# GBATZOLIS/conditional_score_diffusion

Hardware: AMD Instinct MI355X
Metric: images/sec for 1000-step PC sampling, ddpm_paired_SR3 score net of celebA_SR3_160 (BASELINE configs[1]), 160x160 (higher is better)
Workload: dtype f16x3 (every operand carried as hi + lo fp16 = 22 significand bits, 3 MFMAs per product, f32 accumulate; f32-class: the per-op test tolerance is the f32 kernel's, network error 1.9e-6 vs the reference); 1 GPU; BASELINE configs[1]: celebA_SR3_160 (ddpm_paired_SR3, nf=96, ch_mult (1,1,2,2,3,3), attn 20/10/5), 1000-step PC (reverse_diffusion + langevin, snr 0.15), batch 64 per GPU, random-init weights, synthetic LR inputs; images_per_gpu=64, global_batch=64, noise=on-device Philox4x32-10, precision_mode=fp16x3

## Files before the change

### conditional_score_diffusion_amd/csrc/conv_ff.h

```cpp
#pragma once
#include <stdlib.h>

#include <type_traits>

#include "conv_f16_kernel.h"

namespace csd {

typedef unsigned int uint4f __attribute__((ext_vector_type(4)));
typedef int int8v __attribute__((ext_vector_type(8)));
typedef short short2v __attribute__((ext_vector_type(2)));

#define FF_THREADS 256
#define FF_TILE 16
#define FF_PW 18
#define FF_NPATCH (FF_PW * FF_PW)
#define FF_PSB 64
#define FF_RS (FF_PW * FF_PSB + 16)
#define FF_PATCH_BYTES (FF_PW * FF_RS)

struct ConvFFArgs {
  ConvArgs a;
  int B, H, W, C0, C1, Cout;
  int tiles_x, tpi, n_groups, nblocks;
  int nstage;
  int abl;
};

__device__ __forceinline__ void ff_barrier() {
  asm volatile("" ::: "memory");
  __builtin_amdgcn_s_waitcnt(0xC07F);
  __builtin_amdgcn_s_barrier();
  asm volatile("" ::: "memory");
}

template <int N>
__device__ __forceinline__ void ff_wait_vm() {
  asm volatile("s_waitcnt vmcnt(%0)" ::"n"(N) : "memory");
}

template <int NS, int NT>
struct FFCfg {
  static constexpr int KC = NS == 1 ? 32 : 16;
  static constexpr int KSUB = NS == 1 ? 2 : 1;
  static constexpr int STEPS = KSUB * 9;
  static constexpr int TG = NS == 1 ? 2 : 1;
  static constexpr int GPS = STEPS / TG;
  static constexpr int SB = NT * NS * 1024;
  static constexpr int GB = TG * SB;
  static constexpr int GL = GB / 1024;
  static constexpr int R = 5;
  static constexpr int G4 = KC / 4;
  static constexpr int NDMA = 1;
  static constexpr int GLW = GL / NDMA;
  static constexpr int LOADERS = (4 - NDMA) * 64;
  static constexpr int NSLOT = (FF_NPATCH * G4 + LOADERS - 1) / LOADERS;
  static constexpr int PPJ = LOADERS / G4;
  static constexpr size_t LDS = 2 * (size_t)FF_PATCH_BYTES + (size_t)R * GB + 2 * FF_NPATCH * sizeof(int);
};

int convfx_launch(const ConvFFArgs& k, int nt, hipStream_t s);
bool convxk_supported(const ConvFFArgs& k, int nt);
int convxk_launch(const ConvFFArgs& k, int nt, hipStream_t s);

}
```

### conditional_score_diffusion_amd/csrc/conv_xk.hip

```cpp
#include "conv_ff.h"

#include <utility>

namespace csd {

#define XW_THREADS 256
#define XW_RS (32 * 64 + 16)
#define XW_PATCH_BYTES (FF_PW * XW_RS)
#define XW_NU 162

template <int NT_>
struct XKCfg {
  static constexpr int NT = NT_;
  static constexpr int NA = 4 * NT;
  static constexpr int GP = 3 * NA;
  static constexpr int TAPB = 4 * NT * 2 * 1024;
  static constexpr int STB = 3 * TAPB;
  static constexpr int WPT = 2 * NT;
  static constexpr int XTOG = 65536;
  static constexpr int SLOTB = NT * 1024;
  static constexpr int OFF_X23 = XW_PATCH_BYTES, OFF_DUMMY = OFF_X23 + 8 * SLOTB, OFF_Y0 = XTOG + XW_PATCH_BYTES, OFF_Y8 = 2 * XTOG;
  static constexpr int OFF_RED = OFF_Y8 + 8 * SLOTB;
  static constexpr size_t LDS = (size_t)OFF_RED + 4 * NT * 32 * 2 * sizeof(float);
  static_assert(OFF_DUMMY + 3072 <= XTOG && OFF_Y0 + 8 * SLOTB <= OFF_DUMMY + XTOG && OFF_DUMMY + XTOG + 3072 <= OFF_Y8 && 8 * SLOTB <= XW_PATCH_BYTES &&
                    LDS <= 160 * 1024,
                "conv_xk: LDS map");
};

template <class F, int... I>
__device__ __forceinline__ void xk_static_for_impl(F&& f, std::integer_sequence<int, I...>) {
  (f(std::integral_constant<int, I>{}), ...);
}
template <int N, class F>
__device__ __forceinline__ void xk_static_for(F&& f) {
  xk_static_for_impl(static_cast<F&&>(f), std::make_integer_sequence<int, N>{});
}

typedef unsigned int xk_u4 __attribute__((ext_vector_type(4)));

__device__ __forceinline__ int xk_pack_f16(float a, float b) {
  typedef float f2 __attribute__((ext_vector_type(2)));
  typedef _Float16 h2 __attribute__((ext_vector_type(2)));
  return __builtin_bit_cast(int, __builtin_convertvector(f2{a, b}, h2));
}
template <bool HIGH>
__device__ __forceinline__ float xk_lo(int hp, float v) {
  float r;
  if constexpr (HIGH) asm("v_fma_mix_f32 %0, %1, -1.0, %2 op_sel:[1,0,0] op_sel_hi:[1,0,0]" : "=v"(r) : "v"(hp), "v"(v));
  else asm("v_fma_mix_f32 %0, %1, -1.0, %2 op_sel_hi:[1,0,0]" : "=v"(r) : "v"(hp), "v"(v));
  return r;
}

#define XW_FENCE() __builtin_amdgcn_sched_barrier(0)
#define XW_SADD(x, y) asm volatile("s_add_u32 %0, %0, %1" : "+s"(x) : "s"(y) : "scc")
#define XW_PIN(a) asm volatile("" : "+v"(a))
#ifndef XK_ABL
#define XK_ABL 0
#endif
#ifdef CSD_FF_TUNE
#define XW_WALL(i) do { if (a_dbg && tid == 0) a_dbg[blockIdx.x * 32 + (i)] = wall_clock64(); } while (0)
#else
#define XW_WALL(i) do { } while (0)
#endif

template <int NT>
struct XKSched {
  static constexpr int PB = 4 * NT, GP = 3 * PB, WPT = 2 * NT;
  static constexpr bool rd_xl(int g) { return g < PB && g % NT == NT - 1; }
  static constexpr bool rd_xh(int g) { return g >= 2 * PB && g % NT == NT - 1; }
  static constexpr bool slot_req(int g) { return g == 0; }
  static constexpr bool ld_w(int g) { return g >= PB && g < PB + WPT; }
  static constexpr int fixed(int g) { return (rd_xl(g) ? 1 : 0) + (rd_xh(g) ? 1 : 0) + (ld_w(g) ? 1 : 0) + (slot_req(g) ? 3 : 0); }
  static constexpr int wgt(int g) { return 14 - 3 * fixed(g) > 2 ? 14 - 3 * fixed(g) : 2; }
  static constexpr int cum(int g) { int s = 0; for (int h = 0; h < g; ++h) s += wgt(h); return s; }
  static constexpr int first_op(int n, int g) { return (int)(((long long)n * cum(g)) / cum(GP)); }
};

template <int NT_, bool NORM, bool RES>
__global__ __launch_bounds__(XW_THREADS, 1) void conv_xk_kernel(const char* __restrict__ g_wpack, const ConvFFArgs k) {
  using C = XKCfg<NT_>;
  using S = XKSched<NT_>;
  constexpr int NT = C::NT, NA = C::NA, GP = C::GP, TAPB = C::TAPB, STB = C::STB, WPT = C::WPT, PB = S::PB;
  constexpr int OFF_RED = C::OFF_RED, OFF_DUMMY = C::OFF_DUMMY, XTOG = C::XTOG, SLOTB = C::SLOTB;
  extern __shared__ __attribute__((aligned(16))) char smem[];

  const float* const a_src0 = k.a.src0;
  const float* const a_src1 = k.a.src1;
  const float* const a_bias = k.a.bias;
  const float* const a_temb = k.a.temb;
  const float* const a_res = k.a.res;
  float* const a_out = k.a.out;
  double* const a_stats = k.a.stats;
  const int a_temb_stride = k.a.temb_stride, a_out_stride = k.a.out_stride, a_out_coff = k.a.out_coff;
  const float a_out_scale = k.a.out_scale;
  const int kH = k.H, kW = k.W, kC0 = k.C0, kC1 = k.C1, kCout = k.Cout, k_tiles_x = k.tiles_x, k_tpi = k.tpi,
            k_n_groups = k.n_groups, k_nblocks = k.nblocks, NS = k.nstage;
  const int Cin = kC0 + kC1;

  const int tid = threadIdx.x;
  const int lane = tid & 63;
  const int wave = __builtin_amdgcn_readfirstlane(tid >> 6);
  const int kh = lane >> 5, p32 = lane & 31, lg = lane & 3, ul = lane >> 2;
#ifdef CSD_FF_TUNE
  long long* const a_dbg = k.a.dbg;
#endif
  XW_WALL(30);

  const int xcd = blockIdx.x & 7, wj = blockIdx.x >> 3, wstride = gridDim.x >> 3;
  const int xq = k_nblocks >> 3, xr = k_nblocks & 7;
  const int x_start = xcd < xr ? xcd * (xq + 1) : xr * (xq + 1) + (xcd - xr) * xq, x_len = xq + (xcd < xr ? 1 : 0);
  const int n_my = x_len > wj ? (x_len - wj + wstride - 1) / wstride : 0;
  if (n_my == 0) return;
  struct Tile { int ng, b, ty0, tx0, tile; };
  auto tile_at = [&](int it) __attribute__((always_inline)) {
    Tile t;
    it = it < n_my ? it : n_my - 1;
    const int w = x_start + wj + it * wstride;
    t.ng = w % k_n_groups;
    t.tile = w / k_n_groups;
    t.b = t.tile / k_tpi;
    const int tin = t.tile - t.b * k_tpi;
    t.ty0 = (tin / k_tiles_x) * FF_TILE;
    t.tx0 = (tin - (tin / k_tiles_x) * k_tiles_x) * FF_TILE;
    return t;
  };

  auto fresh_lane = [&]() __attribute__((always_inline)) { int l = lane; asm volatile("" : "+v"(l)); return l; };
  constexpr unsigned OOB = 0x80000000u;
  constexpr int RSRC_FLAGS = 0x00020000;
  constexpr float NLOG2E = -1.4426950408889634f;
  const float ka = (NORM ? -0.6931471805599453f / C16_WSCALE : 1.0f / C16_WSCALE) * a_out_scale;

  int s_dst[3];
#pragma unroll
  for (int j = 0; j < 3; ++j) {
    const int U = 15 * (4 * j + wave) + ul;
    const int Uc = U < XW_NU ? U : XW_NU - 1;
    const int pr = Uc / 9, u = Uc - pr * 9;
    const bool writer = U < XW_NU && ul < 15 && u < 8;
    const int rec = pr * XW_RS + u * 64 + lg * 8;
    const int dummy = OFF_DUMMY + ul * 64 + lg * 8;
    s_dst[j] = writer ? rec : dummy;
  }
  struct Geom { int p[3]; };
  auto geom_of = [&](const Tile& t) __attribute__((always_inline)) {
    Geom g;
    const int ulf = fresh_lane() >> 2;
#pragma unroll
    for (int j = 0; j < 3; ++j) {
      const int U = 15 * (4 * j + wave) + ulf;
      const int Uc = U < XW_NU ? U : XW_NU - 1;
      const int pr = Uc / 9, u = Uc - pr * 9;
      const int y = t.ty0 - 1 + pr, xa = t.tx0 - 1 + 2 * u;
      const bool iny = (unsigned)y < (unsigned)kH && U < XW_NU;
      const bool ina = iny && (unsigned)xa < (unsigned)kW, inb = iny && (unsigned)(xa + 1) < (unsigned)kW;
      g.p[j] = (ina ? y * kW + xa : inb ? y * kW + xa + 1 : 0) | (ina ? (int)0x80000000 : 0) | (inb ? 0x40000000 : 0) |
               (ina && inb ? 0x20000000 : 0);
    }
    return g;
  };
  const int nb_addr = ((lane + 4) & 63) * 4;

  const int xbase = (p32 >> 3) * XW_RS + (p32 & 7) * 64 + kh * 16 + wave * 512;
  int xb_cur = xbase, xb_nxt = xbase + XTOG;

  xk_u4 pfa[3], pfb[3];
  xk_u4 scn, shn;
  float msc[4], msh[4];
  __amdgpu_buffer_rsrc_t srcL;
  int strideL = 0, soffL = 0;
  auto src_of = [&](const Tile& t, int st) __attribute__((always_inline)) {
    const int cb = st * 16;
    const bool s1 = cb >= kC0;
    const int Cs = s1 ? kC1 : kC0;
    const float* base = (s1 ? a_src1 : a_src0) + (size_t)t.b * kH * kW * Cs;
    srcL = __builtin_amdgcn_make_buffer_rsrc(const_cast<float*>(base), 0, OOB, RSRC_FLAGS);
    strideL = Cs * 4;
    soffL = (s1 ? cb - kC0 : cb) * 4;
  };
  auto req_a = [&](int j, const Geom& g) __attribute__((always_inline)) {
    if (!(XK_ABL & 16)) pfa[j] = __builtin_amdgcn_raw_buffer_load_b128(srcL, (XK_ABL & 8192) ? (unsigned)(tid * 16 + j * 8192) : __umul24((XK_ABL & 4096) ? (g.p[j] & 255) : g.p[j], strideL) + lg * 16, soffL, 0);
  };
  auto req_b = [&](int j, const Geom& g) __attribute__((always_inline)) {
    if (!(XK_ABL & 16)) pfb[j] = __builtin_amdgcn_raw_buffer_load_b128(srcL, (XK_ABL & 8192) ? (unsigned)(tid * 16 + j * 8192 + 4096) : __umul24(((XK_ABL & 4096) ? (g.p[j] & 255) : g.p[j]) + ((g.p[j] >> 29) & 1), strideL) + lg * 16, soffL, 0);
  };
  const __amdgpu_buffer_rsrc_t nsc_r = __builtin_amdgcn_make_buffer_rsrc(const_cast<float*>(NORM ? k.a.nscale : a_src0), 0, OOB, RSRC_FLAGS);
  const __amdgpu_buffer_rsrc_t nsh_r = __builtin_amdgcn_make_buffer_rsrc(const_cast<float*>(NORM ? k.a.nshift : a_src0), 0, OOB, RSRC_FLAGS);
  auto req_norm = [&](const Tile& t, int st) __attribute__((always_inline)) {
    if constexpr (NORM) {
      const int so = (t.b * Cin + st * 16) * 4;
      scn = __builtin_amdgcn_raw_buffer_load_b128(nsc_r, (unsigned)(lg * 16), so, 0);
      shn = __builtin_amdgcn_raw_buffer_load_b128(nsh_r, (unsigned)(lg * 16), so, 0);
    }
  };
  auto cvt_prep_half = [&](int h) __attribute__((always_inline)) {
    if constexpr (NORM) {
#pragma unroll
      for (int q = 2 * h; q < 2 * h + 2; ++q) {
        msc[q] = __uint_as_float(scn[q]) * NLOG2E;
        msh[q] = __uint_as_float(shn[q]) * NLOG2E;
      }
      asm volatile("" : "+v"(msc[2 * h]), "+v"(msc[2 * h + 1]), "+v"(msh[2 * h]), "+v"(msh[2 * h + 1]));
    }
  };
  const __amdgpu_buffer_rsrc_t w_r = __builtin_amdgcn_make_buffer_rsrc(const_cast<char*>(g_wpack), 0, OOB, RSRC_FLAGS);
  const int wvoff = lane * 16 + wave * (WPT * 1024);
  int w_run = 0;
  const int c_tapb = TAPB;
  auto w_begin = [&](int wso) __attribute__((always_inline)) { w_run = wso; };
  auto w_next_tap = [&]() __attribute__((always_inline)) { XW_SADD(w_run, c_tapb); };

  constexpr int NPH = NORM ? 7 : 2, NPRE = 8 * NPH, NPOST = 24, NMATH = NPRE + 2 * NPOST;
  struct PreOrder {
    int val[8 * 7], ph[8 * 7];
    constexpr PreOrder(int nph) : val{}, ph{} {
      int n = 0;
      for (int d = 0; d < nph + 7; ++d)
        for (int i = 0; i < 8; ++i)
          if (d - i >= 0 && d - i < nph) { val[n] = i; ph[n] = d - i; ++n; }
    }
  };
  constexpr PreOrder PRE(NPH);
  float cv[8], ce[8], cn[8], cd[4][2], cl[4][2];
  int chp[4][2], clp[4][2];
  auto math_op = [&](auto j_tag, auto o_tag, const Geom& g) __attribute__((always_inline)) {
    constexpr int j = decltype(j_tag)::value, ol = decltype(o_tag)::value;
    if (XK_ABL & 1) return;
    if constexpr (ol < NPRE) {
      constexpr int i = PRE.val[ol], c = i & 3, o = PRE.ph[ol] + (NORM ? 0 : 5);
      if constexpr (o == 0) {
        const float x = __uint_as_float(i < 4 ? pfa[j][c] : pfb[j][c]);
        cv[i] = fmaf(x, msc[c], msh[c]);
        XW_PIN(cv[i]);
      } else if constexpr (o == 1) {
        ce[i] = (XK_ABL & 1024) ? cv[i] * 1.5f : __builtin_amdgcn_exp2f(cv[i]);
        XW_PIN(ce[i]);
      } else if constexpr (o == 2) {
        ce[i] = 1.0f + ce[i];
        XW_PIN(ce[i]);
      } else if constexpr (o == 3) {
        ce[i] = (XK_ABL & 1024) ? ce[i] * 0.7f : __builtin_amdgcn_rcpf(ce[i]);
        XW_PIN(ce[i]);
      } else if constexpr (o == 4) {
        cv[i] = cv[i] * ce[i];
        XW_PIN(cv[i]);
      } else if constexpr (o == 5) {
        const int m = (i < 4 ? g.p[j] : g.p[j] << 1) >> 31;
        const int raw = NORM ? __float_as_int(cv[i]) : (int)(i < 4 ? pfa[j][c] : pfb[j][c]);
        cv[i] = __int_as_float(raw & m);
        XW_PIN(cv[i]);
      } else {
        if (XK_ABL & 512) { cn[i] = cv[i] * 0.5f; XW_PIN(cn[i]); }
        else cn[i] = __int_as_float(__builtin_amdgcn_ds_bpermute(nb_addr, __float_as_int(cv[i])));
      }
    } else {
      constexpr int hh = (ol - NPRE) / NPOST, o = (ol - NPRE) % NPOST;
      if constexpr (o < 8) {
        constexpr int kc = o >> 1, c = o & 1, ca = 2 * hh + c, cb = 4 + ca;
        if constexpr (kc == 0) cd[0][c] = cv[ca] - cn[ca];
        else if constexpr (kc == 1) cd[1][c] = cv[cb] + cn[ca];
        else if constexpr (kc == 2) cd[2][c] = cn[ca] - cv[cb];
        else cd[3][c] = cv[cb] - cn[cb];
        XW_PIN(cd[kc][c]);
      } else if constexpr (o < 12) {
        constexpr int kc = o - 8;
        if (XK_ABL & 2048) { chp[kc][hh] = __float_as_int(cd[kc][0]); clp[kc][hh] = __float_as_int(cd[kc][1]); return; }
        chp[kc][hh] = xk_pack_f16(cd[kc][0], cd[kc][1]);
        XW_PIN(chp[kc][hh]);
      } else if constexpr (o < 20) {
        if (XK_ABL & 2048) return;
        constexpr int kc = (o - 12) >> 1, c = (o - 12) & 1;
        if constexpr (c == 0) cl[kc][0] = xk_lo<false>(chp[kc][hh], cd[kc][0]);
        else cl[kc][1] = xk_lo<true>(chp[kc][hh], cd[kc][1]);
        XW_PIN(cl[kc][c]);
      } else {
        if (XK_ABL & 2048) return;
        constexpr int kc = o - 20;
        clp[kc][hh] = xk_pack_f16(cl[kc][0], cl[kc][1]);
        XW_PIN(clp[kc][hh]);
      }
    }
  };
  auto write_op = [&](auto j_tag, auto o_tag) __attribute__((always_inline)) {
    constexpr int j = decltype(j_tag)::value, o = decltype(o_tag)::value;
    if (XK_ABL & (1 | 256)) return;
    constexpr int kc = o & 3, pl = o >> 2;
    char* const rec = smem + s_dst[j] + kc * 512 + pl * 32;
    if constexpr (pl == 0) *reinterpret_cast<int2*>(rec) = make_int2(chp[kc][0], chp[kc][1]);
    else *reinterpret_cast<int2*>(rec) = make_int2(clp[kc][0], clp[kc][1]);
  };
  auto reqs_op = [&](auto j_tag, auto o_tag, const Geom& g) __attribute__((always_inline)) {
    constexpr int j = decltype(j_tag)::value, o = decltype(o_tag)::value;
    if constexpr (o == 0) req_a(j, g);
    else req_b(j, g);
  };
  using J0 = std::integral_constant<int, 0>;
  using J1 = std::integral_constant<int, 1>;
  using J2 = std::integral_constant<int, 2>;
  constexpr int NFULL = NMATH + 8;
  auto full_op = [&](auto j_tag, auto o_tag, const Geom& gm, const Geom& gr) __attribute__((always_inline)) {
    constexpr int o = decltype(o_tag)::value;
    if constexpr (o < NMATH) math_op(j_tag, o_tag, gm);
    else write_op(j_tag, std::integral_constant<int, o - NMATH>{});
  };

  half8 xh[4], xl[4], w0[WPT], w1[WPT], w2[WPT];
  auto rd_x = [&](half8& dst, int xb, int r, int m, int pl) __attribute__((always_inline)) {
    if (XK_ABL & 4) return;
    dst = *reinterpret_cast<const half8*>(smem + xb + (4 * m + r) * XW_RS + pl * 32);
  };
  auto ld_w = [&](half8& dst, int i) __attribute__((always_inline)) {
    if (XK_ABL & 2) return;
    dst = __builtin_bit_cast(half8, __builtin_amdgcn_raw_buffer_load_b128(w_r, (unsigned)(wvoff + i * 1024), w_run, 0));
  };

  floatx16 acc[4][NT];
#define XK_MFMA_AV(ACC, A, B) asm volatile("v_mfma_f32_32x32x16_f16 %0, %1, %2, %0" : "+a"(ACC) : "a"(A), "v"(B))
#define XK_MFMA_AA(ACC, A, B) asm volatile("v_mfma_f32_32x32x16_f16 %0, %1, %2, %0" : "+a"(ACC) : "a"(A), "a"(B))
  auto mm0 = [&](int p, int i) __attribute__((always_inline)) {
    const int m = i / NT, nt = i - m * NT, wi = 2 * nt + (p == 2 ? 1 : 0);
    if (p == 0) XK_MFMA_AV(acc[m][nt], xl[m], w0[wi]); else XK_MFMA_AV(acc[m][nt], xh[m], w0[wi]);
  };
  auto mm1 = [&](int p, int i) __attribute__((always_inline)) {
    const int m = i / NT, nt = i - m * NT, wi = 2 * nt + (p == 2 ? 1 : 0);
    if (p == 0) XK_MFMA_AV(acc[m][nt], xl[m], w1[wi]); else XK_MFMA_AV(acc[m][nt], xh[m], w1[wi]);
  };
  auto mm2 = [&](int p, int i) __attribute__((always_inline)) {
    const int m = i / NT, nt = i - m * NT, wi = 2 * nt + (p == 2 ? 1 : 0);
    if (p == 0) XK_MFMA_AV(acc[m][nt], xl[m], w2[wi]); else XK_MFMA_AV(acc[m][nt], xh[m], w2[wi]);
  };
  auto mm_first = [&](int i) __attribute__((always_inline)) {
    const int m = i / NT, nt = i - m * NT;
    asm volatile("v_mfma_f32_32x32x16_f16 %0, %1, %2, 0" : "=a"(acc[m][nt]) : "a"(xl[m]), "v"(w0[2 * nt]));
  };
  auto tie_acc_done = [&]() __attribute__((always_inline)) {
    static_assert(NT == 3 || NT == 2, "conv_xk: 96- or 64-cout groups");
    if constexpr (NT == 3)
      asm volatile("s_nop 15\n\ts_nop 7"
                   : "+a"(acc[0][0]), "+a"(acc[0][1]), "+a"(acc[0][2]), "+a"(acc[1][0]), "+a"(acc[1][1]), "+a"(acc[1][2]), "+a"(acc[2][0]),
                     "+a"(acc[2][1]), "+a"(acc[2][2]), "+a"(acc[3][0]), "+a"(acc[3][1]), "+a"(acc[3][2]));
    else
      asm volatile("s_nop 15\n\ts_nop 7"
                   : "+a"(acc[0][0]), "+a"(acc[0][1]), "+a"(acc[1][0]), "+a"(acc[1][1]), "+a"(acc[2][0]), "+a"(acc[2][1]), "+a"(acc[3][0]),
                     "+a"(acc[3][1]));
  };

  float rs[4][8][NT];
  float bv[NT], tv[NT];
  __amdgpu_buffer_rsrc_t res_r, out_r;
  unsigned res_voff = 0, out_voff = 0;
  bool e_valid = true;
  int e_tile = 0, e_ng = 0;
  const int res_col = kCout * 4, res_row = (kW - 7) * kCout * 4, out_col = a_out_stride * 4, out_row = (kW - 7) * a_out_stride * 4;
  int res_run = 0;
  const __amdgpu_buffer_rsrc_t bias_r = __builtin_amdgcn_make_buffer_rsrc(const_cast<float*>(a_bias ? a_bias : a_src0), 0, a_bias ? OOB : 0u, RSRC_FLAGS);
  auto epi_setup = [&](const Tile& t) __attribute__((always_inline)) {
    const size_t tile_pix = (size_t)t.b * kH * kW + (size_t)t.ty0 * kW + t.tx0;
    out_r = __builtin_amdgcn_make_buffer_rsrc(a_out + tile_pix * a_out_stride + a_out_coff, 0, OOB, RSRC_FLAGS);
    e_tile = t.tile; e_ng = t.ng;
    if constexpr (RES) {
      res_r = __builtin_amdgcn_make_buffer_rsrc(const_cast<float*>(a_res + tile_pix * kCout), 0, OOB, RSRC_FLAGS);
      res_run = 0;
    }
  };
  auto epi_loads = [&](const Tile& t) __attribute__((always_inline)) {
    const int lf = fresh_lane();
    const int c_lane = t.ng * NT * 32 + (lf & 31);
    e_valid = (t.ty0 + 4 * wave < kH) && (t.tx0 + 8 * (lf >> 5) < kW);
    out_voff = e_valid ? (unsigned)((4 * wave * kW + 8 * (lf >> 5)) * a_out_stride + c_lane) * 4u : OOB;
    if constexpr (RES) res_voff = e_valid ? (unsigned)((4 * wave * kW + 8 * (lf >> 5)) * kCout + c_lane) * 4u : OOB;
    const __amdgpu_buffer_rsrc_t tb_r = __builtin_amdgcn_make_buffer_rsrc(const_cast<float*>(a_temb ? a_temb + (size_t)t.b * a_temb_stride : a_src0), 0,
                                                                           a_temb ? OOB : 0u, RSRC_FLAGS);
#pragma unroll
    for (int nt = 0; nt < NT; ++nt) {
      bv[nt] = __uint_as_float(__builtin_amdgcn_raw_buffer_load_b32(bias_r, (unsigned)(c_lane + nt * 32) * 4u, 0, 0));
      tv[nt] = __uint_as_float(__builtin_amdgcn_raw_buffer_load_b32(tb_r, (unsigned)(c_lane + nt * 32) * 4u, 0, 0));
    }
  };
  auto req_res = [&](int e) __attribute__((always_inline)) {
    if constexpr (RES) {
      if (XK_ABL & 32) return;
      const int idx = e / NT, nt = e - idx * NT;
      rs[idx >> 3][idx & 7][nt] = __uint_as_float(__builtin_amdgcn_raw_buffer_load_b32(res_r, res_voff + nt * 128, res_run, 0));
      if (nt == NT - 1 && idx < 31) {
        if ((idx & 7) != 7) XW_SADD(res_run, res_col);
        else XW_SADD(res_run, res_row);
      }
    }
  };
  float* const red = reinterpret_cast<float*>(smem + OFF_RED);
  int ex_dead = XTOG;
  auto epilogue = [&]() __attribute__((always_inline)) {
    if constexpr (RES) {
#pragma unroll
      for (int e = 8 * NT; e < 32 * NT; ++e) req_res(e);
    }
    tie_acc_done();
    const int lf = fresh_lane();
    const int l16 = lf * 16;
    const int txX01 = ex_dead + wave * SLOTB + l16, txX23 = C::OFF_X23 + wave * SLOTB + l16;
    const int txY0 = C::OFF_Y0 + wave * SLOTB + l16, txY8 = C::OFF_Y8 + wave * SLOTB + l16;
    const int rxX = (wave < 2 ? ex_dead + wave * 4 * SLOTB : C::OFF_X23 + (wave - 2) * 4 * SLOTB) + l16;
    const int rxY = (wave < 2 ? C::OFF_Y0 + wave * 4 * SLOTB : C::OFF_Y8 + (wave - 2) * 4 * SLOTB) + l16;
    float ps[NT][4], pq[NT][4];
#pragma unroll
    for (int nt = 0; nt < NT; ++nt)
#pragma unroll
      for (int q = 0; q < 4; ++q) ps[nt][q] = pq[nt][q] = 0.f;
    int out_run = 0;
    typedef float xk_f4 __attribute__((ext_vector_type(4)));
    auto send_block = [&](int row, int d) __attribute__((always_inline)) {
      const int tx = (row & 1) ? ((d < 2 ? txY0 : txY8) + (d & 1) * 4 * SLOTB) : ((d < 2 ? txX01 : txX23) + (d & 1) * 4 * SLOTB);
#pragma unroll
      for (int nt = 0; nt < NT; ++nt)
        if (!(XK_ABL & 128))
          *reinterpret_cast<xk_f4*>(smem + tx + nt * 1024) =
              xk_f4{acc[d][nt][4 * row], acc[d][nt][4 * row + 1], acc[d][nt][4 * row + 2], acc[d][nt][4 * row + 3]};
    };
#pragma unroll
    for (int row = 0; row < ((XK_ABL & 524288) ? 0 : 4); ++row) {
      if (row == 0) {
#pragma unroll
        for (int d = 0; d < 4; ++d) send_block(0, d);
      }
      if (!(XK_ABL & 65536)) ff_barrier();
      xk_f4 mv[4][NT];
#pragma unroll
      for (int c = 0; c < 4; ++c)
#pragma unroll
        for (int nt = 0; nt < NT; ++nt) {
          if (XK_ABL & 131072) mv[c][nt] = xk_f4{acc[c][nt][4 * row], acc[c][nt][4 * row + 1], acc[c][nt][4 * row + 2], acc[c][nt][4 * row + 3]};
          else mv[c][nt] = *reinterpret_cast<const xk_f4*>(smem + ((row & 1) ? rxY : rxX) + c * SLOTB + nt * 1024);
        }
#pragma unroll
      for (int jj = 0; jj < 4; ++jj) {
        float y1[NT];
#pragma unroll
        for (int nt = 0; nt < NT; ++nt) {
          const float bs = (bv[nt] + tv[nt]) * a_out_scale;
          const float m0 = mv[0][nt][jj], m1 = mv[1][nt][jj], m2 = mv[2][nt][jj], m3 = mv[3][nt][jj];
          const float y0 = (m0 + m1) + m2;
          y1[nt] = (m1 - m2) - m3;
          float v;
          if constexpr (RES) v = fmaf(y0, ka, fmaf(rs[row][2 * jj][nt], a_out_scale, bs));
          else v = fmaf(y0, ka, bs);
          if (!(XK_ABL & 8)) __builtin_amdgcn_raw_buffer_store_b32(__float_as_uint(v), out_r, out_voff + nt * 128, out_run, 0);
          if (!(XK_ABL & 262144)) { ps[nt][(jj & 1) * 2] += v; pq[nt][(jj & 1) * 2] = fmaf(v, v, pq[nt][(jj & 1) * 2]); }
        }
        XW_SADD(out_run, out_col);
#pragma unroll
        for (int nt = 0; nt < NT; ++nt) {
          const float bs = (bv[nt] + tv[nt]) * a_out_scale;
          float v;
          if constexpr (RES) v = fmaf(y1[nt], ka, fmaf(rs[row][2 * jj + 1][nt], a_out_scale, bs));
          else v = fmaf(y1[nt], ka, bs);
          if (!(XK_ABL & 8)) __builtin_amdgcn_raw_buffer_store_b32(__float_as_uint(v), out_r, out_voff + nt * 128, out_run, 0);
          if (!(XK_ABL & 262144)) { ps[nt][(jj & 1) * 2 + 1] += v; pq[nt][(jj & 1) * 2 + 1] = fmaf(v, v, pq[nt][(jj & 1) * 2 + 1]); }
        }
        if (jj != 3) XW_SADD(out_run, out_col);
        else if (row != 3) XW_SADD(out_run, out_row);
        XW_FENCE();
        if (row < 3) send_block(row + 1, jj);
        XW_FENCE();
      }
    }
    if (a_stats) {
      const int tidf = wave * 64 + lf;
      float vs[NT], vq[NT];
#pragma unroll
      for (int nt = 0; nt < NT; ++nt) {
        vs[nt] = (ps[nt][0] + ps[nt][1]) + (ps[nt][2] + ps[nt][3]);
        vq[nt] = (pq[nt][0] + pq[nt][1]) + (pq[nt][2] + pq[nt][3]);
        vs[nt] = e_valid ? vs[nt] : 0.f;
        vq[nt] = e_valid ? vq[nt] : 0.f;
        vs[nt] += __shfl_xor(vs[nt], 32);
        vq[nt] += __shfl_xor(vq[nt], 32);
        if (lf < 32) {
          red[(wave * NT * 32 + nt * 32 + lf) * 2 + 0] = vs[nt];
          red[(wave * NT * 32 + nt * 32 + lf) * 2 + 1] = vq[nt];
        }
      }
      ff_barrier();
      if (tidf < NT * 32) {
        double sm = 0.0, sq = 0.0;
#pragma unroll
        for (int wv = 0; wv < 4; ++wv) {
          sm += (double)red[(wv * NT * 32 + tidf) * 2 + 0];
          sq += (double)red[(wv * NT * 32 + tidf) * 2 + 1];
        }
        double* dst = a_stats + ((size_t)e_tile * kCout + e_ng * NT * 32 + tidf) * 2;
        dst[0] = sm;
        dst[1] = sq;
      }
    }
  };

  Tile tc = tile_at(0), tn = tile_at(1);
  Geom gc = geom_of(tc), gn = gc;
  const int NSTB = (Cin / 16) * STB;

  src_of(tc, 0);
#pragma unroll
  for (int j = 0; j < 3; ++j) { req_a(j, gc); req_b(j, gc); }
  req_norm(tc, 0);
  w_begin(tc.ng * NSTB);
  {
    cvt_prep_half(0); cvt_prep_half(1);
    req_norm(tc, 1);
    src_of(tc, 1);
    xk_static_for<NFULL>([&](auto o) __attribute__((always_inline)) { full_op(J0{}, o, gc, gc); });
    req_a(0, gc); req_b(0, gc);
    xk_static_for<NFULL>([&](auto o) __attribute__((always_inline)) { full_op(J1{}, o, gc, gc); });
    req_a(1, gc); req_b(1, gc);
    xk_static_for<NFULL>([&](auto o) __attribute__((always_inline)) { full_op(J2{}, o, gc, gc); });
    req_a(2, gc); req_b(2, gc);
#pragma unroll
    for (int j = 0; j < 3; ++j) s_dst[j] ^= XTOG;
    cvt_prep_half(0); cvt_prep_half(1);
    xk_static_for<NMATH>([&](auto o) __attribute__((always_inline)) { math_op(J0{}, o, gc); });
#pragma unroll
    for (int i = 0; i < WPT; ++i) ld_w(w0[i], i);
    w_next_tap();
#pragma unroll
    for (int i = 0; i < WPT; ++i) ld_w(w1[i], i);
    w_next_tap();
  }
  ff_barrier();
#pragma unroll
  for (int m = 0; m < 4; ++m) { rd_x(xh[m], xb_cur, 0, m, 0); rd_x(xl[m], xb_cur, 0, m, 1); }

  auto unit = [&](auto pos_tag, auto first_tag, int s) __attribute__((always_inline)) {
    constexpr int POS = decltype(pos_tag)::value;
    constexpr bool FIRST = decltype(first_tag)::value;
    const Tile& tx = POS == 2 ? tn : tc;
    const Tile& tl = POS >= 1 ? tn : tc;
    const Geom& gx = POS == 2 ? gn : gc;
    const Geom& gl = POS >= 1 ? gn : gc;
    const int sl = POS == 0 ? s + 2 : POS - 1;
    xk_static_for<3>([&](auto r_tag) __attribute__((always_inline)) {
      constexpr int R = decltype(r_tag)::value;
      XW_FENCE();
      if constexpr (R == 2) { if (!(XK_ABL & 64)) ff_barrier(); }
      XW_FENCE();
      if constexpr (R == 0) src_of(tl, sl);
      if constexpr (R == 1 && POS == 2) w_begin(tn.ng * NSTB);
      constexpr int NOPS = R == 0 ? 8 + NFULL : R == 1 ? NFULL : 2 + NMATH;
      xk_static_for<GP>([&](auto g_tag) __attribute__((always_inline)) {
        constexpr int g = decltype(g_tag)::value;
        XW_FENCE();
        if constexpr (FIRST && R == 0 && g < NA) mm_first(g);
        else if constexpr (R == 0) mm0(g / NA, g % NA);
        else if constexpr (R == 1) mm1(g / NA, g % NA);
        else mm2(g / NA, g % NA);
        XW_FENCE();
        if constexpr (S::rd_xl(g)) rd_x(xl[g / NT], R == 2 ? xb_nxt : xb_cur, (R + 1) % 3, g / NT, 1);
        if constexpr (S::rd_xh(g)) rd_x(xh[(g - 2 * PB) / NT], R == 2 ? xb_nxt : xb_cur, (R + 1) % 3, (g - 2 * PB) / NT, 0);
        if constexpr (S::slot_req(g)) { req_a(R, gl); req_b(R, gl); }
        if constexpr (S::ld_w(g)) {
          if constexpr (R == 0) ld_w(w2[g - PB], g - PB);
          else if constexpr (R == 1) ld_w(w0[g - PB], g - PB);
          else ld_w(w1[g - PB], g - PB);
          if constexpr (g == PB + WPT - 1) w_next_tap();
        }
        if constexpr (R == 0 && g == 2 && POS == 1) epi_setup(tc);
        if constexpr (R == 1 && g == PB + PB / 2) req_norm(tl, sl);
        if constexpr (R == 2 && POS == 2 && g == PB) epi_loads(tc);
        constexpr int o0 = S::first_op(NOPS, g), o1 = S::first_op(NOPS, g + 1);
        xk_static_for<o1 - o0>([&](auto d_tag) __attribute__((always_inline)) {
          constexpr int o = o0 + decltype(d_tag)::value;
          if constexpr (R == 0) {
            if constexpr (o < 8) write_op(J0{}, std::integral_constant<int, o>{});
            else full_op(J1{}, std::integral_constant<int, o - 8>{}, gx, gl);
          } else if constexpr (R == 1) {
            full_op(J2{}, std::integral_constant<int, o>{}, gx, gl);
          } else {
            if constexpr (o < 2) cvt_prep_half(o);
            else math_op(J0{}, std::integral_constant<int, o - 2>{}, gl);
          }
        });
        if constexpr (RES && POS == 2 && R == 2 && g >= 2 * PB) {
          constexpr int per = (8 * NT + PB - 1) / PB;
#pragma unroll
          for (int e = (g - 2 * PB) * per; e < (g - 2 * PB + 1) * per && e < 8 * NT; ++e) req_res(e);
        }
      });
    });
    XW_FENCE();
#pragma unroll
    for (int j = 0; j < 3; ++j) s_dst[j] ^= XTOG;
    xb_cur ^= XTOG;
    xb_nxt ^= XTOG;
    ex_dead ^= XTOG;
  };
  using P0 = std::integral_constant<int, 0>;
  using P1 = std::integral_constant<int, 1>;
  using P2 = std::integral_constant<int, 2>;
  using Yes = std::true_type;
  using No = std::false_type;

  for (int it = 0; it < n_my; ++it) {
#ifdef CSD_FF_TUNE
    if (it == 1) XW_WALL(28);
    if (it == 2) XW_WALL(29);
    if (it == 1 && a_dbg && tid == 0) a_dbg[blockIdx.x * 32 + 26] = clock64();
    if (it == 2 && a_dbg && tid == 0) a_dbg[blockIdx.x * 32 + 27] = clock64();
#endif
    unit(P0{}, Yes{}, 0);
    for (int s = 1; s + 2 < NS; ++s) unit(P0{}, No{}, s);
    gn = geom_of(tn);
    unit(P1{}, No{}, NS - 2);
    unit(P2{}, No{}, NS - 1);
    epilogue();
    tc = tn;
    gc = gn;
    tn = tile_at(it + 2);
  }
  XW_WALL(31);
}

template <int NT, bool NORM, bool RES>
static int launch_xk(const ConvFFArgs& k, hipStream_t s) {
  auto kern = conv_xk_kernel<NT, NORM, RES>;
  CSD_SET_MAX_LDS_ONCE(kern);
  const int n_cu = device_cu_count8();
  const int grid = k.nblocks < n_cu ? (k.nblocks + 7) / 8 * 8 : n_cu;
  hipLaunchKernelGGL(kern, dim3(grid), dim3(XW_THREADS), XKCfg<NT>::LDS, s, reinterpret_cast<const char*>(k.a.wpack), k);
  CSD_LAUNCH_CHECK();
  return CSD_OK;
}

bool convxk_supported(const ConvFFArgs& k, int nt) { return (nt == 3 || nt == 2) && k.nstage >= 3; }

int convxk_launch(const ConvFFArgs& k, int nt, hipStream_t s) {
  const bool norm = k.a.nscale != nullptr, res = k.a.res != nullptr;
  if (nt == 2) {
    if (norm) return res ? launch_xk<2, true, true>(k, s) : launch_xk<2, true, false>(k, s);
    return res ? launch_xk<2, false, true>(k, s) : launch_xk<2, false, false>(k, s);
  }
  if (norm) return res ? launch_xk<3, true, true>(k, s) : launch_xk<3, true, false>(k, s);
  return res ? launch_xk<3, false, true>(k, s) : launch_xk<3, false, false>(k, s);
}

}
```

Before: 1.619 images/sec.

## Add half-height tile path to conv_xk for 8-row remainder strips

The conv_xk kernel body moves into an include file instantiated for MT=4 (full 16-row tiles) and MT=2 (half-height tiles). When H mod 16 is 8, as at the 40/10 resolutions, the last tile row is handled by separate workgroups running a half-height walk with a rescheduled op sequence and two prefetch slots. The launcher splits the grid between full and half workers using a cost model. This is meant to avoid computing padded rows that are masked out, at the cost of a more complex schedule, a larger binary and a risk of load imbalance between the two groups.

```diff
diff --git a/conditional_score_diffusion_amd/csrc/conv_ff.h b/conditional_score_diffusion_amd/csrc/conv_ff.h
--- a/conditional_score_diffusion_amd/csrc/conv_ff.h
+++ b/conditional_score_diffusion_amd/csrc/conv_ff.h
@@ -25,6 +25,7 @@
   int tiles_x, tpi, n_groups, nblocks;
   int nstage;
   int abl;
+  int tpi_full, nblocks_full, wg8_full;
 };
 
 __device__ __forceinline__ void ff_barrier() {
diff --git a/conditional_score_diffusion_amd/csrc/conv_xk.hip b/conditional_score_diffusion_amd/csrc/conv_xk.hip
--- a/conditional_score_diffusion_amd/csrc/conv_xk.hip
+++ b/conditional_score_diffusion_amd/csrc/conv_xk.hip
@@ -7,12 +7,13 @@
 #define XW_THREADS 256
 #define XW_RS (32 * 64 + 16)
 #define XW_PATCH_BYTES (FF_PW * XW_RS)
-#define XW_NU 162
 
-template <int NT_>
+template <int NT_, int MT_ = 4>
 struct XKCfg {
-  static constexpr int NT = NT_;
-  static constexpr int NA = 4 * NT;
+  static constexpr int NT = NT_, MT = MT_;
+  static constexpr int NA = MT * NT;
+  static constexpr int NSLOT = MT == 4 ? 3 : 2;
+  static constexpr int NU = 9 * (4 * MT + 2);
   static constexpr int GP = 3 * NA;
   static constexpr int TAPB = 4 * NT * 2 * 1024;
   static constexpr int STB = 3 * TAPB;
@@ -63,9 +64,9 @@
 #define XW_WALL(i) do { } while (0)
 #endif
 
-template <int NT>
+template <int NT, int MT = 4>
 struct XKSched {
-  static constexpr int PB = 4 * NT, GP = 3 * PB, WPT = 2 * NT;
+  static constexpr int PB = MT * NT, GP = 3 * PB, WPT = 2 * NT;
   static constexpr bool rd_xl(int g) { return g < PB && g % NT == NT - 1; }
   static constexpr bool rd_xh(int g) { return g >= 2 * PB && g % NT == NT - 1; }
   static constexpr bool slot_req(int g) { return g == 0; }
@@ -74,557 +75,70 @@
   static constexpr int wgt(int g) { return 14 - 3 * fixed(g) > 2 ? 14 - 3 * fixed(g) : 2; }
   static constexpr int cum(int g) { int s = 0; for (int h = 0; h < g; ++h) s += wgt(h); return s; }
   static constexpr int first_op(int n, int g) { return (int)(((long long)n * cum(g)) / cum(GP)); }
+  static constexpr int first_op3(int n, int r, int g) { return (int)(((long long)n * (r * cum(GP) + cum(g))) / (3 * cum(GP))); }
 };
 
-template <int NT_, bool NORM, bool RES>
+#define XK_MFMA_AV(ACC, A, B) asm volatile("v_mfma_f32_32x32x16_f16 %0, %1, %2, %0" : "+a"(ACC) : "a"(A), "v"(B))
+#define XK_MFMA_AA(ACC, A, B) asm volatile("v_mfma_f32_32x32x16_f16 %0, %1, %2, %0" : "+a"(ACC) : "a"(A), "a"(B))
+
+template <int NT_, int MT_, bool NORM, bool RES>
 __global__ __launch_bounds__(XW_THREADS, 1) void conv_xk_kernel(const char* __restrict__ g_wpack, const ConvFFArgs k) {
-  using C = XKCfg<NT_>;
-  using S = XKSched<NT_>;
-  constexpr int NT = C::NT, NA = C::NA, GP = C::GP, TAPB = C::TAPB, STB = C::STB, WPT = C::WPT, PB = S::PB;
-  constexpr int OFF_RED = C::OFF_RED, OFF_DUMMY = C::OFF_DUMMY, XTOG = C::XTOG, SLOTB = C::SLOTB;
-  extern __shared__ __attribute__((aligned(16))) char smem[];
+  if constexpr (MT_ == 4) {
+#define XK_WALK_MT 4
+#define XK_WALK_SPLIT false
+#include "conv_xk_walk.inc"
+  } else if ((int)(blockIdx.x >> 3) < k.wg8_full) {
+    asm volatile("; conv_xk walk MT = 4");
+#define XK_WALK_MT 4
+#define XK_WALK_SPLIT true
+#include "conv_xk_walk.inc"
+  } else {
+    asm volatile("; conv_xk walk MT = 2");
+#define XK_WALK_MT 2
+#define XK_WALK_SPLIT true
+#include "conv_xk_walk.inc"
+  }
+}
 
-  const float* const a_src0 = k.a.src0;
-  const float* const a_src1 = k.a.src1;
-  const float* const a_bias = k.a.bias;
-  const float* const a_temb = k.a.temb;
-  const float* const a_res = k.a.res;
-  float* const a_out = k.a.out;
-  double* const a_stats = k.a.stats;
-  const int a_temb_stride = k.a.temb_stride, a_out_stride = k.a.out_stride, a_out_coff = k.a.out_coff;
-  const float a_out_scale = k.a.out_scale;
-  const int kH = k.H, kW = k.W, kC0 = k.C0, kC1 = k.C1, kCout = k.Cout, k_tiles_x = k.tiles_x, k_tpi = k.tpi,
-            k_n_groups = k.n_groups, k_nblocks = k.nblocks, NS = k.nstage;
-  const int Cin = kC0 + kC1;
+static constexpr double XK_HALF_COST = 0.67;
 
-  const int tid = threadIdx.x;
-  const int lane = tid & 63;
-  const int wave = __builtin_amdgcn_readfirstlane(tid >> 6);
-  const int kh = lane >> 5, p32 = lane & 31, lg = lane & 3, ul = lane >> 2;
-#ifdef CSD_FF_TUNE
-  long long* const a_dbg = k.a.dbg;
-#endif
-  XW_WALL(30);
+static int xk_rounds(int items, int wg8) { return wg8 > 0 ? ((items + 7) / 8 + wg8 - 1) / wg8 : 0; }
 
-  const int xcd = blockIdx.x & 7, wj = blockIdx.x >> 3, wstride = gridDim.x >> 3;
-  const int xq = k_nblocks >> 3, xr = k_nblocks & 7;
-  const int x_start = xcd < xr ? xcd * (xq + 1) : xr * (xq + 1) + (xcd - xr) * xq, x_len = xq + (xcd < xr ? 1 : 0);
-  const int n_my = x_len > wj ? (x_len - wj + wstride - 1) / wstride : 0;
-  if (n_my == 0) return;
-  struct Tile { int ng, b, ty0, tx0, tile; };
-  auto tile_at = [&](int it) __attribute__((always_inline)) {
-    Tile t;
-    it = it < n_my ? it : n_my - 1;
-    const int w = x_start + wj + it * wstride;
-    t.ng = w % k_n_groups;
-    t.tile = w / k_n_groups;
-    t.b = t.tile / k_tpi;
-    const int tin = t.tile - t.b * k_tpi;
-    t.ty0 = (tin / k_tiles_x) * FF_TILE;
-    t.tx0 = (tin - (tin / k_tiles_x) * k_tiles_x) * FF_TILE;
-    return t;
-  };
-
-  auto fresh_lane = [&]() __attribute__((always_inline)) { int l = lane; asm volatile("" : "+v"(l)); return l; };
-  constexpr unsigned OOB = 0x80000000u;
-  constexpr int RSRC_FLAGS = 0x00020000;
-  constexpr float NLOG2E = -1.4426950408889634f;
-  const float ka = (NORM ? -0.6931471805599453f / C16_WSCALE : 1.0f / C16_WSCALE) * a_out_scale;
-
-  int s_dst[3];
-#pragma unroll
-  for (int j = 0; j < 3; ++j) {
-    const int U = 15 * (4 * j + wave) + ul;
-    const int Uc = U < XW_NU ? U : XW_NU - 1;
-    const int pr = Uc / 9, u = Uc - pr * 9;
-    const bool writer = U < XW_NU && ul < 15 && u < 8;
-    const int rec = pr * XW_RS + u * 64 + lg * 8;
-    const int dummy = OFF_DUMMY + ul * 64 + lg * 8;
-    s_dst[j] = writer ? rec : dummy;
-  }
-  struct Geom { int p[3]; };
-  auto geom_of = [&](const Tile& t) __attribute__((always_inline)) {
-    Geom g;
-    const int ulf = fresh_lane() >> 2;
-#pragma unroll
-    for (int j = 0; j < 3; ++j) {
-      const int U = 15 * (4 * j + wave) + ulf;
-      const int Uc = U < XW_NU ? U : XW_NU - 1;
-      const int pr = Uc / 9, u = Uc - pr * 9;
-      const int y = t.ty0 - 1 + pr, xa = t.tx0 - 1 + 2 * u;
-      const bool iny = (unsigned)y < (unsigned)kH && U < XW_NU;
-      const bool ina = iny && (unsigned)xa < (unsigned)kW, inb = iny && (unsigned)(xa + 1) < (unsigned)kW;
-      g.p[j] = (ina ? y * kW + xa : inb ? y * kW + xa + 1 : 0) | (ina ? (int)0x80000000 : 0) | (inb ? 0x40000000 : 0) |
-               (ina && inb ? 0x20000000 : 0);
-    }
-    return g;
-  };
-  const int nb_addr = ((lane + 4) & 63) * 4;
-
-  const int xbase = (p32 >> 3) * XW_RS + (p32 & 7) * 64 + kh * 16 + wave * 512;
-  int xb_cur = xbase, xb_nxt = xbase + XTOG;
-
-  xk_u4 pfa[3], pfb[3];
-  xk_u4 scn, shn;
-  float msc[4], msh[4];
-  __amdgpu_buffer_rsrc_t srcL;
-  int strideL = 0, soffL = 0;
-  auto src_of = [&](const Tile& t, int st) __attribute__((always_inline)) {
-    const int cb = st * 16;
-    const bool s1 = cb >= kC0;
-    const int Cs = s1 ? kC1 : kC0;
-    const float* base = (s1 ? a_src1 : a_src0) + (size_t)t.b * kH * kW * Cs;
-    srcL = __builtin_amdgcn_make_buffer_rsrc(const_cast<float*>(base), 0, OOB, RSRC_FLAGS);
-    strideL = Cs * 4;
-    soffL = (s1 ? cb - kC0 : cb) * 4;
-  };
-  auto req_a = [&](int j, const Geom& g) __attribute__((always_inline)) {
-    if (!(XK_ABL & 16)) pfa[j] = __builtin_amdgcn_raw_buffer_load_b128(srcL, (XK_ABL & 8192) ? (unsigned)(tid * 16 + j * 8192) : __umul24((XK_ABL & 4096) ? (g.p[j] & 255) : g.p[j], strideL) + lg * 16, soffL, 0);
-  };
-  auto req_b = [&](int j, const Geom& g) __attribute__((always_inline)) {
-    if (!(XK_ABL & 16)) pfb[j] = __builtin_amdgcn_raw_buffer_load_b128(srcL, (XK_ABL & 8192) ? (unsigned)(tid * 16 + j * 8192 + 4096) : __umul24(((XK_ABL & 4096) ? (g.p[j] & 255) : g.p[j]) + ((g.p[j] >> 29) & 1), strideL) + lg * 16, soffL, 0);
-  };
-  const __amdgpu_buffer_rsrc_t nsc_r = __builtin_amdgcn_make_buffer_rsrc(const_cast<float*>(NORM ? k.a.nscale : a_src0), 0, OOB, RSRC_FLAGS);
-  const __amdgpu_buffer_rsrc_t nsh_r = __builtin_amdgcn_make_buffer_rsrc(const_cast<float*>(NORM ? k.a.nshift : a_src0), 0, OOB, RSRC_FLAGS);
-  auto req_norm = [&](const Tile& t, int st) __attribute__((always_inline)) {
-    if constexpr (NORM) {
-      const int so = (t.b * Cin + st * 16) * 4;
-      scn = __builtin_amdgcn_raw_buffer_load_b128(nsc_r, (unsigned)(lg * 16), so, 0);
-      shn = __builtin_amdgcn_raw_buffer_load_b128(nsh_r, (unsigned)(lg * 16), so, 0);
-    }
-  };
-  auto cvt_prep_half = [&](int h) __attribute__((always_inline)) {
-    if constexpr (NORM) {
-#pragma unroll
-      for (int q = 2 * h; q < 2 * h + 2; ++q) {
-        msc[q] = __uint_as_float(scn[q]) * NLOG2E;
-        msh[q] = __uint_as_float(shn[q]) * NLOG2E;
-      }
-      asm volatile("" : "+v"(msc[2 * h]), "+v"(msc[2 * h + 1]), "+v"(msh[2 * h]), "+v"(msh[2 * h + 1]));
-    }
-  };
-  const __amdgpu_buffer_rsrc_t w_r = __builtin_amdgcn_make_buffer_rsrc(const_cast<char*>(g_wpack), 0, OOB, RSRC_FLAGS);
-  const int wvoff = lane * 16 + wave * (WPT * 1024);
-  int w_run = 0;
-  const int c_tapb = TAPB;
-  auto w_begin = [&](int wso) __attribute__((always_inline)) { w_run = wso; };
-  auto w_next_tap = [&]() __attribute__((always_inline)) { XW_SADD(w_run, c_tapb); };
-
-  constexpr int NPH = NORM ? 7 : 2, NPRE = 8 * NPH, NPOST = 24, NMATH = NPRE + 2 * NPOST;
-  struct PreOrder {
-    int val[8 * 7], ph[8 * 7];
-    constexpr PreOrder(int nph) : val{}, ph{} {
-      int n = 0;
-      for (int d = 0; d < nph + 7; ++d)
-        for (int i = 0; i < 8; ++i)
-          if (d - i >= 0 && d - i < nph) { val[n] = i; ph[n] = d - i; ++n; }
-    }
-  };
-  constexpr PreOrder PRE(NPH);
-  float cv[8], ce[8], cn[8], cd[4][2], cl[4][2];
-  int chp[4][2], clp[4][2];
-  auto math_op = [&](auto j_tag, auto o_tag, const Geom& g) __attribute__((always_inline)) {
-    constexpr int j = decltype(j_tag)::value, ol = decltype(o_tag)::value;
-    if (XK_ABL & 1) return;
-    if constexpr (ol < NPRE) {
-      constexpr int i = PRE.val[ol], c = i & 3, o = PRE.ph[ol] + (NORM ? 0 : 5);
-      if constexpr (o == 0) {
-        const float x = __uint_as_float(i < 4 ? pfa[j][c] : pfb[j][c]);
-        cv[i] = fmaf(x, msc[c], msh[c]);
-        XW_PIN(cv[i]);
-      } else if constexpr (o == 1) {
-        ce[i] = (XK_ABL & 1024) ? cv[i] * 1.5f : __builtin_amdgcn_exp2f(cv[i]);
-        XW_PIN(ce[i]);
-      } else if constexpr (o == 2) {
-        ce[i] = 1.0f + ce[i];
-        XW_PIN(ce[i]);
-      } else if constexpr (o == 3) {
-        ce[i] = (XK_ABL & 1024) ? ce[i] * 0.7f : __builtin_amdgcn_rcpf(ce[i]);
-        XW_PIN(ce[i]);
-      } else if constexpr (o == 4) {
-        cv[i] = cv[i] * ce[i];
-        XW_PIN(cv[i]);
-      } else if constexpr (o == 5) {
-        const int m = (i < 4 ? g.p[j] : g.p[j] << 1) >> 31;
-        const int raw = NORM ? __float_as_int(cv[i]) : (int)(i < 4 ? pfa[j][c] : pfb[j][c]);
-        cv[i] = __int_as_float(raw & m);
-        XW_PIN(cv[i]);
-      } else {
-        if (XK_ABL & 512) { cn[i] = cv[i] * 0.5f; XW_PIN(cn[i]); }
-        else cn[i] = __int_as_float(__builtin_amdgcn_ds_bpermute(nb_addr, __float_as_int(cv[i])));
-      }
+template <int NT, bool NORM, bool RES>
+static int launch_xk(const ConvFFArgs& k0, hipStream_t s) {
+  ConvFFArgs k = k0;
+  const int n_cu = device_cu_count8();
+  int grid = k.nblocks < n_cu ? (k.nblocks + 7) / 8 * 8 : n_cu;
+  k.tpi_full = k.tpi; k.nblocks_full = k.nblocks; k.wg8_full = grid / 8;
+  bool half = NT == 3 && k.H % FF_TILE == 8 && !CSD_TUNE_ENV("CSD_XK_NO_HALF");
+  if (half) {
+    k.tpi_full = k.tpi - k.tiles_x;
+    k.nblocks_full = k.B * k.tpi_full * k.n_groups;
+    const int n_half = k.nblocks - k.nblocks_full;
+    const int g8f = (k.nblocks_full + 7) / 8, g8h = (n_half + 7) / 8;
+    if (8 * (g8f + g8h) <= n_cu) {
+      k.wg8_full = g8f;
+      grid = 8 * (g8f + g8h);
     } else {
-      constexpr int hh = (ol - NPRE) / NPOST, o = (ol - NPRE) % NPOST;
-      if constexpr (o < 8) {
-        constexpr int kc = o >> 1, c = o & 1, ca = 2 * hh + c, cb = 4 + ca;
-        if constexpr (kc == 0) cd[0][c] = cv[ca] - cn[ca];
-        else if constexpr (kc == 1) cd[1][c] = cv[cb] + cn[ca];
-        else if constexpr (kc == 2) cd[2][c] = cn[ca] - cv[cb];
-        else cd[3][c] = cv[cb] - cn[cb];
-        XW_PIN(cd[kc][c]);
-      } else if constexpr (o < 12) {
-        constexpr int kc = o - 8;
-        if (XK_ABL & 2048) { chp[kc][hh] = __float_as_int(cd[kc][0]); clp[kc][hh] = __float_as_int(cd[kc][1]); return; }
-        chp[kc][hh] = xk_pack_f16(cd[kc][0], cd[kc][1]);
-        XW_PIN(chp[kc][hh]);
-      } else if constexpr (o < 20) {
-        if (XK_ABL & 2048) return;
-        constexpr int kc = (o - 12) >> 1, c = (o - 12) & 1;
-        if constexpr (c == 0) cl[kc][0] = xk_lo<false>(chp[kc][hh], cd[kc][0]);
-        else cl[kc][1] = xk_lo<true>(chp[kc][hh], cd[kc][1]);
-        XW_PIN(cl[kc][c]);
-      } else {
-        if (XK_ABL & 2048) return;
-        constexpr int kc = o - 20;
-        clp[kc][hh] = xk_pack_f16(cl[kc][0], cl[kc][1]);
-        XW_PIN(clp[kc][hh]);
+      double best = 0.0;
+      for (int h8 = 1; h8 < grid / 8; ++h8) {
+        const double tf = xk_rounds(k.nblocks_full, grid / 8 - h8), th = XK_HALF_COST * xk_rounds(n_half, h8);
+        const double t = tf > th ? tf : th;
+        if (h8 == 1 || t < best) { best = t; k.wg8_full = grid / 8 - h8; }
       }
     }
-  };
-  auto write_op = [&](auto j_tag, auto o_tag) __attribute__((always_inline)) {
-    constexpr int j = decltype(j_tag)::value, o = decltype(o_tag)::value;
-    if (XK_ABL & (1 | 256)) return;
-    constexpr int kc = o & 3, pl = o >> 2;
-    char* const rec = smem + s_dst[j] + kc * 512 + pl * 32;
-    if constexpr (pl == 0) *reinterpret_cast<int2*>(rec) = make_int2(chp[kc][0], chp[kc][1]);
-    else *reinterpret_cast<int2*>(rec) = make_int2(clp[kc][0], clp[kc][1]);
-  };
-  auto reqs_op = [&](auto j_tag, auto o_tag, const Geom& g) __attribute__((always_inline)) {
-    constexpr int j = decltype(j_tag)::value, o = decltype(o_tag)::value;
-    if constexpr (o == 0) req_a(j, g);
-    else req_b(j, g);
-  };
-  using J0 = std::integral_constant<int, 0>;
-  using J1 = std::integral_constant<int, 1>;
-  using J2 = std::integral_constant<int, 2>;
-  constexpr int NFULL = NMATH + 8;
-  auto full_op = [&](auto j_tag, auto o_tag, const Geom& gm, const Geom& gr) __attribute__((always_inline)) {
-    constexpr int o = decltype(o_tag)::value;
-    if constexpr (o < NMATH) math_op(j_tag, o_tag, gm);
-    else write_op(j_tag, std::integral_constant<int, o - NMATH>{});
-  };
-
-  half8 xh[4], xl[4], w0[WPT], w1[WPT], w2[WPT];
-  auto rd_x = [&](half8& dst, int xb, int r, int m, int pl) __attribute__((always_inline)) {
-    if (XK_ABL & 4) return;
-    dst = *reinterpret_cast<const half8*>(smem + xb + (4 * m + r) * XW_RS + pl * 32);
-  };
-  auto ld_w = [&](half8& dst, int i) __attribute__((always_inline)) {
-    if (XK_ABL & 2) return;
-    dst = __builtin_bit_cast(half8, __builtin_amdgcn_raw_buffer_load_b128(w_r, (unsigned)(wvoff + i * 1024), w_run, 0));
-  };
-
-  floatx16 acc[4][NT];
-#define XK_MFMA_AV(ACC, A, B) asm volatile("v_mfma_f32_32x32x16_f16 %0, %1, %2, %0" : "+a"(ACC) : "a"(A), "v"(B))
-#define XK_MFMA_AA(ACC, A, B) asm volatile("v_mfma_f32_32x32x16_f16 %0, %1, %2, %0" : "+a"(ACC) : "a"(A), "a"(B))
-  auto mm0 = [&](int p, int i) __attribute__((always_inline)) {
-    const int m = i / NT, nt = i - m * NT, wi = 2 * nt + (p == 2 ? 1 : 0);
-    if (p == 0) XK_MFMA_AV(acc[m][nt], xl[m], w0[wi]); else XK_MFMA_AV(acc[m][nt], xh[m], w0[wi]);
-  };
-  auto mm1 = [&](int p, int i) __attribute__((always_inline)) {
-    const int m = i / NT, nt = i - m * NT, wi = 2 * nt + (p == 2 ? 1 : 0);
-    if (p == 0) XK_MFMA_AV(acc[m][nt], xl[m], w1[wi]); else XK_MFMA_AV(acc[m][nt], xh[m], w1[wi]);
-  };
-  auto mm2 = [&](int p, int i) __attribute__((always_inline)) {
-    const int m = i / NT, nt = i - m * NT, wi = 2 * nt + (p == 2 ? 1 : 0);
-    if (p == 0) XK_MFMA_AV(acc[m][nt], xl[m], w2[wi]); else XK_MFMA_AV(acc[m][nt], xh[m], w2[wi]);
-  };
-  auto mm_first = [&](int i) __attribute__((always_inline)) {
-    const int m = i / NT, nt = i - m * NT;
-    asm volatile("v_mfma_f32_32x32x16_f16 %0, %1, %2, 0" : "=a"(acc[m][nt]) : "a"(xl[m]), "v"(w0[2 * nt]));
-  };
-  auto tie_acc_done = [&]() __attribute__((always_inline)) {
-    static_assert(NT == 3 || NT == 2, "conv_xk: 96- or 64-cout groups");
-    if constexpr (NT == 3)
-      asm volatile("s_nop 15\n\ts_nop 7"
-                   : "+a"(acc[0][0]), "+a"(acc[0][1]), "+a"(acc[0][2]), "+a"(acc[1][0]), "+a"(acc[1][1]), "+a"(acc[1][2]), "+a"(acc[2][0]),
-                     "+a"(acc[2][1]), "+a"(acc[2][2]), "+a"(acc[3][0]), "+a"(acc[3][1]), "+a"(acc[3][2]));
-    else
-      asm volatile("s_nop 15\n\ts_nop 7"
-                   : "+a"(acc[0][0]), "+a"(acc[0][1]), "+a"(acc[1][0]), "+a"(acc[1][1]), "+a"(acc[2][0]), "+a"(acc[2][1]), "+a"(acc[3][0]),
-                     "+a"(acc[3][1]));
-  };
-
-  float rs[4][8][NT];
-  float bv[NT], tv[NT];
-  __amdgpu_buffer_rsrc_t res_r, out_r;
-  unsigned res_voff = 0, out_voff = 0;
-  bool e_valid = true;
-  int e_tile = 0, e_ng = 0;
-  const int res_col = kCout * 4, res_row = (kW - 7) * kCout * 4, out_col = a_out_stride * 4, out_row = (kW - 7) * a_out_stride * 4;
-  int res_run = 0;
-  const __amdgpu_buffer_rsrc_t bias_r = __builtin_amdgcn_make_buffer_rsrc(const_cast<float*>(a_bias ? a_bias : a_src0), 0, a_bias ? OOB : 0u, RSRC_FLAGS);
-  auto epi_setup = [&](const Tile& t) __attribute__((always_inline)) {
-    const size_t tile_pix = (size_t)t.b * kH * kW + (size_t)t.ty0 * kW + t.tx0;
-    out_r = __builtin_amdgcn_make_buffer_rsrc(a_out + tile_pix * a_out_stride + a_out_coff, 0, OOB, RSRC_FLAGS);
-    e_tile = t.tile; e_ng = t.ng;
-    if constexpr (RES) {
-      res_r = __builtin_amdgcn_make_buffer_rsrc(const_cast<float*>(a_res + tile_pix * kCout), 0, OOB, RSRC_FLAGS);
-      res_run = 0;
+  }
+  if (half) {
+    if constexpr (NT == 3) {
+      auto kern = conv_xk_kernel<NT, 2, NORM, RES>;
+      CSD_SET_MAX_LDS_ONCE(kern);
+      hipLaunchKernelGGL(kern, dim3(grid), dim3(XW_THREADS), XKCfg<NT>::LDS, s, reinterpret_cast<const char*>(k.a.wpack), k);
     }
-  };
-  auto epi_loads = [&](const Tile& t) __attribute__((always_inline)) {
-    const int lf = fresh_lane();
-    const int c_lane = t.ng * NT * 32 + (lf & 31);
-    e_valid = (t.ty0 + 4 * wave < kH) && (t.tx0 + 8 * (lf >> 5) < kW);
-    out_voff = e_valid ? (unsigned)((4 * wave * kW + 8 * (lf >> 5)) * a_out_stride + c_lane) * 4u : OOB;
-    if constexpr (RES) res_voff = e_valid ? (unsigned)((4 * wave * kW + 8 * (lf >> 5)) * kCout + c_lane) * 4u : OOB;
-    const __amdgpu_buffer_rsrc_t tb_r = __builtin_amdgcn_make_buffer_rsrc(const_cast<float*>(a_temb ? a_temb + (size_t)t.b * a_temb_stride : a_src0), 0,
-                                                                           a_temb ? OOB : 0u, RSRC_FLAGS);
-#pragma unroll
-    for (int nt = 0; nt < NT; ++nt) {
-      bv[nt] = __uint_as_float(__builtin_amdgcn_raw_buffer_load_b32(bias_r, (unsigned)(c_lane + nt * 32) * 4u, 0, 0));
-      tv[nt] = __uint_as_float(__builtin_amdgcn_raw_buffer_load_b32(tb_r, (unsigned)(c_lane + nt * 32) * 4u, 0, 0));
-    }
-  };
-  auto req_res = [&](int e) __attribute__((always_inline)) {
-    if constexpr (RES) {
-      if (XK_ABL & 32) return;
-      const int idx = e / NT, nt = e - idx * NT;
-      rs[idx >> 3][idx & 7][nt] = __uint_as_float(__builtin_amdgcn_raw_buffer_load_b32(res_r, res_voff + nt * 128, res_run, 0));
-      if (nt == NT - 1 && idx < 31) {
-        if ((idx & 7) != 7) XW_SADD(res_run, res_col);
-        else XW_SADD(res_run, res_row);
-      }
-    }
-  };
-  float* const red = reinterpret_cast<float*>(smem + OFF_RED);
-  int ex_dead = XTOG;
-  auto epilogue = [&]() __attribute__((always_inline)) {
-    if constexpr (RES) {
-#pragma unroll
-      for (int e = 8 * NT; e < 32 * NT; ++e) req_res(e);
-    }
-    tie_acc_done();
-    const int lf = fresh_lane();
-    const int l16 = lf * 16;
-    const int txX01 = ex_dead + wave * SLOTB + l16, txX23 = C::OFF_X23 + wave * SLOTB + l16;
-    const int txY0 = C::OFF_Y0 + wave * SLOTB + l16, txY8 = C::OFF_Y8 + wave * SLOTB + l16;
-    const int rxX = (wave < 2 ? ex_dead + wave * 4 * SLOTB : C::OFF_X23 + (wave - 2) * 4 * SLOTB) + l16;
-    const int rxY = (wave < 2 ? C::OFF_Y0 + wave * 4 * SLOTB : C::OFF_Y8 + (wave - 2) * 4 * SLOTB) + l16;
-    float ps[NT][4], pq[NT][4];
-#pragma unroll
-    for (int nt = 0; nt < NT; ++nt)
-#pragma unroll
-      for (int q = 0; q < 4; ++q) ps[nt][q] = pq[nt][q] = 0.f;
-    int out_run = 0;
-    typedef float xk_f4 __attribute__((ext_vector_type(4)));
-    auto send_block = [&](int row, int d) __attribute__((always_inline)) {
-      const int tx = (row & 1) ? ((d < 2 ? txY0 : txY8) + (d & 1) * 4 * SLOTB) : ((d < 2 ? txX01 : txX23) + (d & 1) * 4 * SLOTB);
-#pragma unroll
-      for (int nt = 0; nt < NT; ++nt)
-        if (!(XK_ABL & 128))
-          *reinterpret_cast<xk_f4*>(smem + tx + nt * 1024) =
-              xk_f4{acc[d][nt][4 * row], acc[d][nt][4 * row + 1], acc[d][nt][4 * row + 2], acc[d][nt][4 * row + 3]};
-    };
-#pragma unroll
-    for (int row = 0; row < ((XK_ABL & 524288) ? 0 : 4); ++row) {
-      if (row == 0) {
-#pragma unroll
-        for (int d = 0; d < 4; ++d) send_block(0, d);
-      }
-      if (!(XK_ABL & 65536)) ff_barrier();
-      xk_f4 mv[4][NT];
-#pragma unroll
-      for (int c = 0; c < 4; ++c)
-#pragma unroll
-        for (int nt = 0; nt < NT; ++nt) {
-          if (XK_ABL & 131072) mv[c][nt] = xk_f4{acc[c][nt][4 * row], acc[c][nt][4 * row + 1], acc[c][nt][4 * row + 2], acc[c][nt][4 * row + 3]};
-          else mv[c][nt] = *reinterpret_cast<const xk_f4*>(smem + ((row & 1) ? rxY : rxX) + c * SLOTB + nt * 1024);
-        }
-#pragma unroll
-      for (int jj = 0; jj < 4; ++jj) {
-        float y1[NT];
-#pragma unroll
-        for (int nt = 0; nt < NT; ++nt) {
-          const float bs = (bv[nt] + tv[nt]) * a_out_scale;
-          const float m0 = mv[0][nt][jj], m1 = mv[1][nt][jj], m2 = mv[2][nt][jj], m3 = mv[3][nt][jj];
-          const float y0 = (m0 + m1) + m2;
-          y1[nt] = (m1 - m2) - m3;
-          float v;
-          if constexpr (RES) v = fmaf(y0, ka, fmaf(rs[row][2 * jj][nt], a_out_scale, bs));
-          else v = fmaf(y0, ka, bs);
-          if (!(XK_ABL & 8)) __builtin_amdgcn_raw_buffer_store_b32(__float_as_uint(v), out_r, out_voff + nt * 128, out_run, 0);
-          if (!(XK_ABL & 262144)) { ps[nt][(jj & 1) * 2] += v; pq[nt][(jj & 1) * 2] = fmaf(v, v, pq[nt][(jj & 1) * 2]); }
-        }
-        XW_SADD(out_run, out_col);
-#pragma unroll
-        for (int nt = 0; nt < NT; ++nt) {
-          const float bs = (bv[nt] + tv[nt]) * a_out_scale;
-          float v;
-          if constexpr (RES) v = fmaf(y1[nt], ka, fmaf(rs[row][2 * jj + 1][nt], a_out_scale, bs));
-          else v = fmaf(y1[nt], ka, bs);
-          if (!(XK_ABL & 8)) __builtin_amdgcn_raw_buffer_store_b32(__float_as_uint(v), out_r, out_voff + nt * 128, out_run, 0);
-          if (!(XK_ABL & 262144)) { ps[nt][(jj & 1) * 2 + 1] += v; pq[nt][(jj & 1) * 2 + 1] = fmaf(v, v, pq[nt][(jj & 1) * 2 + 1]); }
-        }
-        if (jj != 3) XW_SADD(out_run, out_col);
-        else if (row != 3) XW_SADD(out_run, out_row);
-        XW_FENCE();
-        if (row < 3) send_block(row + 1, jj);
-        XW_FENCE();
-      }
-    }
-    if (a_stats) {
-      const int tidf = wave * 64 + lf;
-      float vs[NT], vq[NT];
-#pragma unroll
-      for (int nt = 0; nt < NT; ++nt) {
-        vs[nt] = (ps[nt][0] + ps[nt][1]) + (ps[nt][2] + ps[nt][3]);
-        vq[nt] = (pq[nt][0] + pq[nt][1]) + (pq[nt][2] + pq[nt][3]);
-        vs[nt] = e_valid ? vs[nt] : 0.f;
-        vq[nt] = e_valid ? vq[nt] : 0.f;
-        vs[nt] += __shfl_xor(vs[nt], 32);
-        vq[nt] += __shfl_xor(vq[nt], 32);
-        if (lf < 32) {
-          red[(wave * NT * 32 + nt * 32 + lf) * 2 + 0] = vs[nt];
-          red[(wave * NT * 32 + nt * 32 + lf) * 2 + 1] = vq[nt];
-        }
-      }
-      ff_barrier();
-      if (tidf < NT * 32) {
-        double sm = 0.0, sq = 0.0;
-#pragma unroll
-        for (int wv = 0; wv < 4; ++wv) {
-          sm += (double)red[(wv * NT * 32 + tidf) * 2 + 0];
-          sq += (double)red[(wv * NT * 32 + tidf) * 2 + 1];
-        }
-        double* dst = a_stats + ((size_t)e_tile * kCout + e_ng * NT * 32 + tidf) * 2;
-        dst[0] = sm;
-        dst[1] = sq;
-      }
-    }
-  };
-
-  Tile tc = tile_at(0), tn = tile_at(1);
-  Geom gc = geom_of(tc), gn = gc;
-  const int NSTB = (Cin / 16) * STB;
-
-  src_of(tc, 0);
-#pragma unroll
-  for (int j = 0; j < 3; ++j) { req_a(j, gc); req_b(j, gc); }
-  req_norm(tc, 0);
-  w_begin(tc.ng * NSTB);
-  {
-    cvt_prep_half(0); cvt_prep_half(1);
-    req_norm(tc, 1);
-    src_of(tc, 1);
-    xk_static_for<NFULL>([&](auto o) __attribute__((always_inline)) { full_op(J0{}, o, gc, gc); });
-    req_a(0, gc); req_b(0, gc);
-    xk_static_for<NFULL>([&](auto o) __attribute__((always_inline)) { full_op(J1{}, o, gc, gc); });
-    req_a(1, gc); req_b(1, gc);
-    xk_static_for<NFULL>([&](auto o) __attribute__((always_inline)) { full_op(J2{}, o, gc, gc); });
-    req_a(2, gc); req_b(2, gc);
-#pragma unroll
-    for (int j = 0; j < 3; ++j) s_dst[j] ^= XTOG;
-    cvt_prep_half(0); cvt_prep_half(1);
-    xk_static_for<NMATH>([&](auto o) __attribute__((always_inline)) { math_op(J0{}, o, gc); });
-#pragma unroll
-    for (int i = 0; i < WPT; ++i) ld_w(w0[i], i);
-    w_next_tap();
-#pragma unroll
-    for (int i = 0; i < WPT; ++i) ld_w(w1[i], i);
-    w_next_tap();
+  } else {
+    auto kern = conv_xk_kernel<NT, 4, NORM, RES>;
+    CSD_SET_MAX_LDS_ONCE(kern);
+    hipLaunchKernelGGL(kern, dim3(grid), dim3(XW_THREADS), XKCfg<NT>::LDS, s, reinterpret_cast<const char*>(k.a.wpack), k);
   }
-  ff_barrier();
-#pragma unroll
-  for (int m = 0; m < 4; ++m) { rd_x(xh[m], xb_cur, 0, m, 0); rd_x(xl[m], xb_cur, 0, m, 1); }
-
-  auto unit = [&](auto pos_tag, auto first_tag, int s) __attribute__((always_inline)) {
-    constexpr int POS = decltype(pos_tag)::value;
-    constexpr bool FIRST = decltype(first_tag)::value;
-    const Tile& tx = POS == 2 ? tn : tc;
-    const Tile& tl = POS >= 1 ? tn : tc;
-    const Geom& gx = POS == 2 ? gn : gc;
-    const Geom& gl = POS >= 1 ? gn : gc;
-    const int sl = POS == 0 ? s + 2 : POS - 1;
-    xk_static_for<3>([&](auto r_tag) __attribute__((always_inline)) {
-      constexpr int R = decltype(r_tag)::value;
-      XW_FENCE();
-      if constexpr (R == 2) { if (!(XK_ABL & 64)) ff_barrier(); }
-      XW_FENCE();
-      if constexpr (R == 0) src_of(tl, sl);
-      if constexpr (R == 1 && POS == 2) w_begin(tn.ng * NSTB);
-      constexpr int NOPS = R == 0 ? 8 + NFULL : R == 1 ? NFULL : 2 + NMATH;
-      xk_static_for<GP>([&](auto g_tag) __attribute__((always_inline)) {
-        constexpr int g = decltype(g_tag)::value;
-        XW_FENCE();
-        if constexpr (FIRST && R == 0 && g < NA) mm_first(g);
-        else if constexpr (R == 0) mm0(g / NA, g % NA);
-        else if constexpr (R == 1) mm1(g / NA, g % NA);
-        else mm2(g / NA, g % NA);
-        XW_FENCE();
-        if constexpr (S::rd_xl(g)) rd_x(xl[g / NT], R == 2 ? xb_nxt : xb_cur, (R + 1) % 3, g / NT, 1);
-        if constexpr (S::rd_xh(g)) rd_x(xh[(g - 2 * PB) / NT], R == 2 ? xb_nxt : xb_cur, (R + 1) % 3, (g - 2 * PB) / NT, 0);
-        if constexpr (S::slot_req(g)) { req_a(R, gl); req_b(R, gl); }
-        if constexpr (S::ld_w(g)) {
-          if constexpr (R == 0) ld_w(w2[g - PB], g - PB);
-          else if constexpr (R == 1) ld_w(w0[g - PB], g - PB);
-          else ld_w(w1[g - PB], g - PB);
-          if constexpr (g == PB + WPT - 1) w_next_tap();
-        }
-        if constexpr (R == 0 && g == 2 && POS == 1) epi_setup(tc);
-        if constexpr (R == 1 && g == PB + PB / 2) req_norm(tl, sl);
-        if constexpr (R == 2 && POS == 2 && g == PB) epi_loads(tc);
-        constexpr int o0 = S::first_op(NOPS, g), o1 = S::first_op(NOPS, g + 1);
-        xk_static_for<o1 - o0>([&](auto d_tag) __attribute__((always_inline)) {
-          constexpr int o = o0 + decltype(d_tag)::value;
-          if constexpr (R == 0) {
-            if constexpr (o < 8) write_op(J0{}, std::integral_constant<int, o>{});
-            else full_op(J1{}, std::integral_constant<int, o - 8>{}, gx, gl);
-          } else if constexpr (R == 1) {
-            full_op(J2{}, std::integral_constant<int, o>{}, gx, gl);
-          } else {
-            if constexpr (o < 2) cvt_prep_half(o);
-            else math_op(J0{}, std::integral_constant<int, o - 2>{}, gl);
-          }
-        });
-        if constexpr (RES && POS == 2 && R == 2 && g >= 2 * PB) {
-          constexpr int per = (8 * NT + PB - 1) / PB;
-#pragma unroll
-          for (int e = (g - 2 * PB) * per; e < (g - 2 * PB + 1) * per && e < 8 * NT; ++e) req_res(e);
-        }
-      });
-    });
-    XW_FENCE();
-#pragma unroll
-    for (int j = 0; j < 3; ++j) s_dst[j] ^= XTOG;
-    xb_cur ^= XTOG;
-    xb_nxt ^= XTOG;
-    ex_dead ^= XTOG;
-  };
-  using P0 = std::integral_constant<int, 0>;
-  using P1 = std::integral_constant<int, 1>;
-  using P2 = std::integral_constant<int, 2>;
-  using Yes = std::true_type;
-  using No = std::false_type;
-
-  for (int it = 0; it < n_my; ++it) {
-#ifdef CSD_FF_TUNE
-    if (it == 1) XW_WALL(28);
-    if (it == 2) XW_WALL(29);
-    if (it == 1 && a_dbg && tid == 0) a_dbg[blockIdx.x * 32 + 26] = clock64();
-    if (it == 2 && a_dbg && tid == 0) a_dbg[blockIdx.x * 32 + 27] = clock64();
-#endif
-    unit(P0{}, Yes{}, 0);
-    for (int s = 1; s + 2 < NS; ++s) unit(P0{}, No{}, s);
-    gn = geom_of(tn);
-    unit(P1{}, No{}, NS - 2);
-    unit(P2{}, No{}, NS - 1);
-    epilogue();
-    tc = tn;
-    gc = gn;
-    tn = tile_at(it + 2);
-  }
-  XW_WALL(31);
-}
-
-template <int NT, bool NORM, bool RES>
-static int launch_xk(const ConvFFArgs& k, hipStream_t s) {
-  auto kern = conv_xk_kernel<NT, NORM, RES>;
-  CSD_SET_MAX_LDS_ONCE(kern);
-  const int n_cu = device_cu_count8();
-  const int grid = k.nblocks < n_cu ? (k.nblocks + 7) / 8 * 8 : n_cu;
-  hipLaunchKernelGGL(kern, dim3(grid), dim3(XW_THREADS), XKCfg<NT>::LDS, s, reinterpret_cast<const char*>(k.a.wpack), k);
   CSD_LAUNCH_CHECK();
   return CSD_OK;
 }
diff --git a/conditional_score_diffusion_amd/csrc/conv_xk_walk.inc b/conditional_score_diffusion_amd/csrc/conv_xk_walk.inc
--- /dev/null
+++ b/conditional_score_diffusion_amd/csrc/conv_xk_walk.inc
@@ -0,0 +1,572 @@
+{
+  using C = XKCfg<NT_, XK_WALK_MT>;
+  using S = XKSched<NT_, XK_WALK_MT>;
+  constexpr bool SPLIT = XK_WALK_SPLIT;
+  constexpr int NT = C::NT, MT = C::MT, NA = C::NA, GP = C::GP, TAPB = C::TAPB, STB = C::STB, WPT = C::WPT, PB = S::PB, NSLOT = C::NSLOT, NU = C::NU;
+  static_assert(MT == 4 || MT == 2, "conv_xk: 16- or 8-row tiles");
+  constexpr int OFF_RED = C::OFF_RED, OFF_DUMMY = C::OFF_DUMMY, XTOG = C::XTOG, SLOTB = C::SLOTB;
+  extern __shared__ __attribute__((aligned(16))) char smem[];
+
+  const float* const a_src0 = k.a.src0;
+  const float* const a_src1 = k.a.src1;
+  const float* const a_bias = k.a.bias;
+  const float* const a_temb = k.a.temb;
+  const float* const a_res = k.a.res;
+  float* const a_out = k.a.out;
+  double* const a_stats = k.a.stats;
+  const int a_temb_stride = k.a.temb_stride, a_out_stride = k.a.out_stride, a_out_coff = k.a.out_coff;
+  const float a_out_scale = k.a.out_scale;
+  const int kH = k.H, kW = k.W, kC0 = k.C0, kC1 = k.C1, kCout = k.Cout, k_tiles_x = k.tiles_x, k_tpi = k.tpi,
+            k_n_groups = k.n_groups, k_nblocks = k.nblocks, NS = k.nstage;
+  const int Cin = kC0 + kC1;
+
+  const int tid = threadIdx.x;
+  const int lane = tid & 63;
+  const int wave = __builtin_amdgcn_readfirstlane(tid >> 6);
+  const int kh = lane >> 5, p32 = lane & 31, lg = lane & 3, ul = lane >> 2;
+#ifdef CSD_FF_TUNE
+  long long* const a_dbg = k.a.dbg;
+#endif
+  XW_WALL(30);
+
+  const int xcd = blockIdx.x & 7;
+  int wj = blockIdx.x >> 3, wstride = gridDim.x >> 3, w_items = k_nblocks, w_tpi = k_tpi, w_tin0 = 0;
+  if constexpr (SPLIT && MT == 4) { wstride = k.wg8_full; w_items = k.nblocks_full; w_tpi = k.tpi_full; }
+  if constexpr (SPLIT && MT == 2) { wj -= k.wg8_full; wstride -= k.wg8_full; w_items -= k.nblocks_full; w_tpi -= k.tpi_full; w_tin0 = k.tpi_full; }
+  const int xq = w_items >> 3, xr = w_items & 7;
+  const int x_start = xcd < xr ? xcd * (xq + 1) : xr * (xq + 1) + (xcd - xr) * xq, x_len = xq + (xcd < xr ? 1 : 0);
+  const int n_my = x_len > wj ? (x_len - wj + wstride - 1) / wstride : 0;
+  if (n_my == 0) return;
+  struct Tile { int ng, b, ty0, tx0, tile; };
+  auto tile_at = [&](int it) __attribute__((always_inline)) {
+    Tile t;
+    it = it < n_my ? it : n_my - 1;
+    const int w = x_start + wj + it * wstride;
+    t.ng = w % k_n_groups;
+    t.tile = w / k_n_groups;
+    int tin;
+    if constexpr (SPLIT) {
+      t.b = t.tile / w_tpi;
+      tin = w_tin0 + t.tile - t.b * w_tpi;
+      t.tile = t.b * k_tpi + tin;
+    } else {
+      t.b = t.tile / k_tpi;
+      tin = t.tile - t.b * k_tpi;
+    }
+    t.ty0 = (tin / k_tiles_x) * FF_TILE;
+    t.tx0 = (tin - (tin / k_tiles_x) * k_tiles_x) * FF_TILE;
+    return t;
+  };
+
+  auto fresh_lane = [&]() __attribute__((always_inline)) { int l = lane; asm volatile("" : "+v"(l)); return l; };
+  constexpr unsigned OOB = 0x80000000u;
+  constexpr int RSRC_FLAGS = 0x00020000;
+  constexpr float NLOG2E = -1.4426950408889634f;
+  const float ka = (NORM ? -0.6931471805599453f / C16_WSCALE : 1.0f / C16_WSCALE) * a_out_scale;
+
+  int s_dst[NSLOT];
+#pragma unroll
+  for (int j = 0; j < NSLOT; ++j) {
+    const int U = 15 * (4 * j + wave) + ul;
+    const int Uc = U < NU ? U : NU - 1;
+    const int pr = Uc / 9, u = Uc - pr * 9;
+    const bool writer = U < NU && ul < 15 && u < 8;
+    const int rec = pr * XW_RS + u * 64 + lg * 8;
+    const int dummy = OFF_DUMMY + ul * 64 + lg * 8;
+    s_dst[j] = writer ? rec : dummy;
+  }
+  struct Geom { int p[NSLOT]; };
+  auto geom_of = [&](const Tile& t) __attribute__((always_inline)) {
+    Geom g;
+    const int ulf = fresh_lane() >> 2;
+#pragma unroll
+    for (int j = 0; j < NSLOT; ++j) {
+      const int U = 15 * (4 * j + wave) + ulf;
+      const int Uc = U < NU ? U : NU - 1;
+      const int pr = Uc / 9, u = Uc - pr * 9;
+      const int y = t.ty0 - 1 + pr, xa = t.tx0 - 1 + 2 * u;
+      const bool iny = (unsigned)y < (unsigned)kH && U < NU;
+      const bool ina = iny && (unsigned)xa < (unsigned)kW, inb = iny && (unsigned)(xa + 1) < (unsigned)kW;
+      g.p[j] = (ina ? y * kW + xa : inb ? y * kW + xa + 1 : 0) | (ina ? (int)0x80000000 : 0) | (inb ? 0x40000000 : 0) |
+               (ina && inb ? 0x20000000 : 0);
+    }
+    return g;
+  };
+  const int nb_addr = ((lane + 4) & 63) * 4;
+
+  const int xbase = (p32 >> 3) * XW_RS + (p32 & 7) * 64 + kh * 16 + wave * 512;
+  int xb_cur = xbase, xb_nxt = xbase + XTOG;
+
+  xk_u4 pfa[NSLOT], pfb[NSLOT];
+  xk_u4 scn, shn;
+  float msc[4], msh[4];
+  __amdgpu_buffer_rsrc_t srcL;
+  int strideL = 0, soffL = 0;
+  auto src_of = [&](const Tile& t, int st) __attribute__((always_inline)) {
+    const int cb = st * 16;
+    const bool s1 = cb >= kC0;
+    const int Cs = s1 ? kC1 : kC0;
+    const float* base = (s1 ? a_src1 : a_src0) + (size_t)t.b * kH * kW * Cs;
+    srcL = __builtin_amdgcn_make_buffer_rsrc(const_cast<float*>(base), 0, OOB, RSRC_FLAGS);
+    strideL = Cs * 4;
+    soffL = (s1 ? cb - kC0 : cb) * 4;
+  };
+  auto req_a = [&](int j, const Geom& g) __attribute__((always_inline)) {
+    if (!(XK_ABL & 16)) pfa[j] = __builtin_amdgcn_raw_buffer_load_b128(srcL, (XK_ABL & 8192) ? (unsigned)(tid * 16 + j * 8192) : __umul24((XK_ABL & 4096) ? (g.p[j] & 255) : g.p[j], strideL) + lg * 16, soffL, 0);
+  };
+  auto req_b = [&](int j, const Geom& g) __attribute__((always_inline)) {
+    if (!(XK_ABL & 16)) pfb[j] = __builtin_amdgcn_raw_buffer_load_b128(srcL, (XK_ABL & 8192) ? (unsigned)(tid * 16 + j * 8192 + 4096) : __umul24(((XK_ABL & 4096) ? (g.p[j] & 255) : g.p[j]) + ((g.p[j] >> 29) & 1), strideL) + lg * 16, soffL, 0);
+  };
+  const __amdgpu_buffer_rsrc_t nsc_r = __builtin_amdgcn_make_buffer_rsrc(const_cast<float*>(NORM ? k.a.nscale : a_src0), 0, OOB, RSRC_FLAGS);
+  const __amdgpu_buffer_rsrc_t nsh_r = __builtin_amdgcn_make_buffer_rsrc(const_cast<float*>(NORM ? k.a.nshift : a_src0), 0, OOB, RSRC_FLAGS);
+  auto req_norm = [&](const Tile& t, int st) __attribute__((always_inline)) {
+    if constexpr (NORM) {
+      const int so = (t.b * Cin + st * 16) * 4;
+      scn = __builtin_amdgcn_raw_buffer_load_b128(nsc_r, (unsigned)(lg * 16), so, 0);
+      shn = __builtin_amdgcn_raw_buffer_load_b128(nsh_r, (unsigned)(lg * 16), so, 0);
+    }
+  };
+  auto cvt_prep_half = [&](int h) __attribute__((always_inline)) {
+    if constexpr (NORM) {
+#pragma unroll
+      for (int q = 2 * h; q < 2 * h + 2; ++q) {
+        msc[q] = __uint_as_float(scn[q]) * NLOG2E;
+        msh[q] = __uint_as_float(shn[q]) * NLOG2E;
+      }
+      asm volatile("" : "+v"(msc[2 * h]), "+v"(msc[2 * h + 1]), "+v"(msh[2 * h]), "+v"(msh[2 * h + 1]));
+    }
+  };
+  const __amdgpu_buffer_rsrc_t w_r = __builtin_amdgcn_make_buffer_rsrc(const_cast<char*>(g_wpack), 0, OOB, RSRC_FLAGS);
+  const int wvoff = lane * 16 + wave * (WPT * 1024);
+  int w_run = 0;
+  const int c_tapb = TAPB;
+  auto w_begin = [&](int wso) __attribute__((always_inline)) { w_run = wso; };
+  auto w_next_tap = [&]() __attribute__((always_inline)) { XW_SADD(w_run, c_tapb); };
+
+  constexpr int NPH = NORM ? 7 : 2, NPRE = 8 * NPH, NPOST = 24, NMATH = NPRE + 2 * NPOST;
+  struct PreOrder {
+    int val[8 * 7], ph[8 * 7];
+    constexpr PreOrder(int nph) : val{}, ph{} {
+      int n = 0;
+      for (int d = 0; d < nph + 7; ++d)
+        for (int i = 0; i < 8; ++i)
+          if (d - i >= 0 && d - i < nph) { val[n] = i; ph[n] = d - i; ++n; }
+    }
+  };
+  constexpr PreOrder PRE(NPH);
+  float cv[8], ce[8], cn[8], cd[4][2], cl[4][2];
+  int chp[4][2], clp[4][2];
+  auto math_op = [&](auto j_tag, auto o_tag, const Geom& g) __attribute__((always_inline)) {
+    constexpr int j = decltype(j_tag)::value, ol = decltype(o_tag)::value;
+    if (XK_ABL & 1) return;
+    if constexpr (ol < NPRE) {
+      constexpr int i = PRE.val[ol], c = i & 3, o = PRE.ph[ol] + (NORM ? 0 : 5);
+      if constexpr (o == 0) {
+        const float x = __uint_as_float(i < 4 ? pfa[j][c] : pfb[j][c]);
+        cv[i] = fmaf(x, msc[c], msh[c]);
+        XW_PIN(cv[i]);
+      } else if constexpr (o == 1) {
+        ce[i] = (XK_ABL & 1024) ? cv[i] * 1.5f : __builtin_amdgcn_exp2f(cv[i]);
+        XW_PIN(ce[i]);
+      } else if constexpr (o == 2) {
+        ce[i] = 1.0f + ce[i];
+        XW_PIN(ce[i]);
+      } else if constexpr (o == 3) {
+        ce[i] = (XK_ABL & 1024) ? ce[i] * 0.7f : __builtin_amdgcn_rcpf(ce[i]);
+        XW_PIN(ce[i]);
+      } else if constexpr (o == 4) {
+        cv[i] = cv[i] * ce[i];
+        XW_PIN(cv[i]);
+      } else if constexpr (o == 5) {
+        const int m = (i < 4 ? g.p[j] : g.p[j] << 1) >> 31;
+        const int raw = NORM ? __float_as_int(cv[i]) : (int)(i < 4 ? pfa[j][c] : pfb[j][c]);
+        cv[i] = __int_as_float(raw & m);
+        XW_PIN(cv[i]);
+      } else {
+        if (XK_ABL & 512) { cn[i] = cv[i] * 0.5f; XW_PIN(cn[i]); }
+        else cn[i] = __int_as_float(__builtin_amdgcn_ds_bpermute(nb_addr, __float_as_int(cv[i])));
+      }
+    } else {
+      constexpr int hh = (ol - NPRE) / NPOST, o = (ol - NPRE) % NPOST;
+      if constexpr (o < 8) {
+        constexpr int kc = o >> 1, c = o & 1, ca = 2 * hh + c, cb = 4 + ca;
+        if constexpr (kc == 0) cd[0][c] = cv[ca] - cn[ca];
+        else if constexpr (kc == 1) cd[1][c] = cv[cb] + cn[ca];
+        else if constexpr (kc == 2) cd[2][c] = cn[ca] - cv[cb];
+        else cd[3][c] = cv[cb] - cn[cb];
+        XW_PIN(cd[kc][c]);
+      } else if constexpr (o < 12) {
+        constexpr int kc = o - 8;
+        if (XK_ABL & 2048) { chp[kc][hh] = __float_as_int(cd[kc][0]); clp[kc][hh] = __float_as_int(cd[kc][1]); return; }
+        chp[kc][hh] = xk_pack_f16(cd[kc][0], cd[kc][1]);
+        XW_PIN(chp[kc][hh]);
+      } else if constexpr (o < 20) {
+        if (XK_ABL & 2048) return;
+        constexpr int kc = (o - 12) >> 1, c = (o - 12) & 1;
+        if constexpr (c == 0) cl[kc][0] = xk_lo<false>(chp[kc][hh], cd[kc][0]);
+        else cl[kc][1] = xk_lo<true>(chp[kc][hh], cd[kc][1]);
+        XW_PIN(cl[kc][c]);
+      } else {
+        if (XK_ABL & 2048) return;
+        constexpr int kc = o - 20;
+        clp[kc][hh] = xk_pack_f16(cl[kc][0], cl[kc][1]);
+        XW_PIN(clp[kc][hh]);
+      }
+    }
+  };
+  auto write_op = [&](auto j_tag, auto o_tag) __attribute__((always_inline)) {
+    constexpr int j = decltype(j_tag)::value, o = decltype(o_tag)::value;
+    if (XK_ABL & (1 | 256)) return;
+    constexpr int kc = o & 3, pl = o >> 2;
+    char* const rec = smem + s_dst[j] + kc * 512 + pl * 32;
+    if constexpr (pl == 0) *reinterpret_cast<int2*>(rec) = make_int2(chp[kc][0], chp[kc][1]);
+    else *reinterpret_cast<int2*>(rec) = make_int2(clp[kc][0], clp[kc][1]);
+  };
+  auto reqs_op = [&](auto j_tag, auto o_tag, const Geom& g) __attribute__((always_inline)) {
+    constexpr int j = decltype(j_tag)::value, o = decltype(o_tag)::value;
+    if constexpr (o == 0) req_a(j, g);
+    else req_b(j, g);
+  };
+  using J0 = std::integral_constant<int, 0>;
+  using J1 = std::integral_constant<int, 1>;
+  using J2 = std::integral_constant<int, 2>;
+  constexpr int NFULL = NMATH + 8;
+  auto full_op = [&](auto j_tag, auto o_tag, const Geom& gm, const Geom& gr) __attribute__((always_inline)) {
+    constexpr int o = decltype(o_tag)::value;
+    if constexpr (o < NMATH) math_op(j_tag, o_tag, gm);
+    else write_op(j_tag, std::integral_constant<int, o - NMATH>{});
+  };
+
+  half8 xh[MT], xl[MT], w0[WPT], w1[WPT], w2[WPT];
+  auto rd_x = [&](half8& dst, int xb, int r, int m, int pl) __attribute__((always_inline)) {
+    if (XK_ABL & 4) return;
+    dst = *reinterpret_cast<const half8*>(smem + xb + (4 * m + r) * XW_RS + pl * 32);
+  };
+  auto ld_w = [&](half8& dst, int i) __attribute__((always_inline)) {
+    if (XK_ABL & 2) return;
+    dst = __builtin_bit_cast(half8, __builtin_amdgcn_raw_buffer_load_b128(w_r, (unsigned)(wvoff + i * 1024), w_run, 0));
+  };
+
+  floatx16 acc[MT][NT];
+  auto mm0 = [&](int p, int i) __attribute__((always_inline)) {
+    const int m = i / NT, nt = i - m * NT, wi = 2 * nt + (p == 2 ? 1 : 0);
+    if (p == 0) XK_MFMA_AV(acc[m][nt], xl[m], w0[wi]); else XK_MFMA_AV(acc[m][nt], xh[m], w0[wi]);
+  };
+  auto mm1 = [&](int p, int i) __attribute__((always_inline)) {
+    const int m = i / NT, nt = i - m * NT, wi = 2 * nt + (p == 2 ? 1 : 0);
+    if (p == 0) XK_MFMA_AV(acc[m][nt], xl[m], w1[wi]); else XK_MFMA_AV(acc[m][nt], xh[m], w1[wi]);
+  };
+  auto mm2 = [&](int p, int i) __attribute__((always_inline)) {
+    const int m = i / NT, nt = i - m * NT, wi = 2 * nt + (p == 2 ? 1 : 0);
+    if (p == 0) XK_MFMA_AV(acc[m][nt], xl[m], w2[wi]); else XK_MFMA_AV(acc[m][nt], xh[m], w2[wi]);
+  };
+  auto mm_first = [&](int i) __attribute__((always_inline)) {
+    const int m = i / NT, nt = i - m * NT;
+    asm volatile("v_mfma_f32_32x32x16_f16 %0, %1, %2, 0" : "=a"(acc[m][nt]) : "a"(xl[m]), "v"(w0[2 * nt]));
+  };
+  auto tie_acc_done = [&]() __attribute__((always_inline)) {
+    static_assert(NT == 3 || NT == 2, "conv_xk: 96- or 64-cout groups");
+    if constexpr (NT == 3 && MT == 4)
+      asm volatile("s_nop 15\n\ts_nop 7"
+                   : "+a"(acc[0][0]), "+a"(acc[0][1]), "+a"(acc[0][2]), "+a"(acc[1][0]), "+a"(acc[1][1]), "+a"(acc[1][2]), "+a"(acc[2][0]),
+                     "+a"(acc[2][1]), "+a"(acc[2][2]), "+a"(acc[3][0]), "+a"(acc[3][1]), "+a"(acc[3][2]));
+    else if constexpr (NT == 3)
+      asm volatile("s_nop 15\n\ts_nop 7" : "+a"(acc[0][0]), "+a"(acc[0][1]), "+a"(acc[0][2]), "+a"(acc[1][0]), "+a"(acc[1][1]), "+a"(acc[1][2]));
+    else if constexpr (MT == 2)
+      asm volatile("s_nop 15\n\ts_nop 7" : "+a"(acc[0][0]), "+a"(acc[0][1]), "+a"(acc[1][0]), "+a"(acc[1][1]));
+    else
+      asm volatile("s_nop 15\n\ts_nop 7"
+                   : "+a"(acc[0][0]), "+a"(acc[0][1]), "+a"(acc[1][0]), "+a"(acc[1][1]), "+a"(acc[2][0]), "+a"(acc[2][1]), "+a"(acc[3][0]),
+                     "+a"(acc[3][1]));
+  };
+
+  float rs[4][8][NT];
+  float bv[NT], tv[NT];
+  __amdgpu_buffer_rsrc_t res_r, out_r;
+  unsigned res_voff = 0, out_voff = 0;
+  bool e_valid = true;
+  int e_tile = 0, e_ng = 0;
+  const int res_col = kCout * 4, res_row = (kW - 7) * kCout * 4, out_col = a_out_stride * 4, out_row = (kW - 7) * a_out_stride * 4;
+  int res_run = 0;
+  const __amdgpu_buffer_rsrc_t bias_r = __builtin_amdgcn_make_buffer_rsrc(const_cast<float*>(a_bias ? a_bias : a_src0), 0, a_bias ? OOB : 0u, RSRC_FLAGS);
+  auto epi_setup = [&](const Tile& t) __attribute__((always_inline)) {
+    const size_t tile_pix = (size_t)t.b * kH * kW + (size_t)t.ty0 * kW + t.tx0;
+    out_r = __builtin_amdgcn_make_buffer_rsrc(a_out + tile_pix * a_out_stride + a_out_coff, 0, OOB, RSRC_FLAGS);
+    e_tile = t.tile; e_ng = t.ng;
+    if constexpr (RES) {
+      res_r = __builtin_amdgcn_make_buffer_rsrc(const_cast<float*>(a_res + tile_pix * kCout), 0, OOB, RSRC_FLAGS);
+      res_run = 0;
+    }
+  };
+  auto epi_loads = [&](const Tile& t) __attribute__((always_inline)) {
+    const int lf = fresh_lane();
+    const int c_lane = t.ng * NT * 32 + (lf & 31);
+    e_valid = (t.ty0 + 4 * wave < kH) && (t.tx0 + 8 * (lf >> 5) < kW);
+    out_voff = e_valid ? (unsigned)((4 * wave * kW + 8 * (lf >> 5)) * a_out_stride + c_lane) * 4u : OOB;
+    if constexpr (RES) res_voff = e_valid ? (unsigned)((4 * wave * kW + 8 * (lf >> 5)) * kCout + c_lane) * 4u : OOB;
+    const __amdgpu_buffer_rsrc_t tb_r = __builtin_amdgcn_make_buffer_rsrc(const_cast<float*>(a_temb ? a_temb + (size_t)t.b * a_temb_stride : a_src0), 0,
+                                                                           a_temb ? OOB : 0u, RSRC_FLAGS);
+#pragma unroll
+    for (int nt = 0; nt < NT; ++nt) {
+      bv[nt] = __uint_as_float(__builtin_amdgcn_raw_buffer_load_b32(bias_r, (unsigned)(c_lane + nt * 32) * 4u, 0, 0));
+      tv[nt] = __uint_as_float(__builtin_amdgcn_raw_buffer_load_b32(tb_r, (unsigned)(c_lane + nt * 32) * 4u, 0, 0));
+    }
+  };
+  auto req_res = [&](int e) __attribute__((always_inline)) {
+    if constexpr (RES) {
+      if (XK_ABL & 32) return;
+      const int idx = e / NT, nt = e - idx * NT;
+      rs[idx >> 3][idx & 7][nt] = __uint_as_float(__builtin_amdgcn_raw_buffer_load_b32(res_r, res_voff + nt * 128, res_run, 0));
+      if (nt == NT - 1 && idx < 31) {
+        if ((idx & 7) != 7) XW_SADD(res_run, res_col);
+        else XW_SADD(res_run, res_row);
+      }
+    }
+  };
+  float* const red = reinterpret_cast<float*>(smem + OFF_RED);
+  int ex_dead = XTOG;
+  auto epilogue = [&]() __attribute__((always_inline)) {
+    if constexpr (RES) {
+#pragma unroll
+      for (int e = 8 * NT; e < 32 * NT; ++e) req_res(e);
+    }
+    tie_acc_done();
+    const int lf = fresh_lane();
+    const int l16 = lf * 16;
+    const int txX01 = ex_dead + wave * SLOTB + l16, txX23 = C::OFF_X23 + wave * SLOTB + l16;
+    const int txY0 = C::OFF_Y0 + wave * SLOTB + l16, txY8 = C::OFF_Y8 + wave * SLOTB + l16;
+    const int rxX = (wave < 2 ? ex_dead + wave * 4 * SLOTB : C::OFF_X23 + (wave - 2) * 4 * SLOTB) + l16;
+    const int rxY = (wave < 2 ? C::OFF_Y0 + wave * 4 * SLOTB : C::OFF_Y8 + (wave - 2) * 4 * SLOTB) + l16;
+    float ps[NT][4], pq[NT][4];
+#pragma unroll
+    for (int nt = 0; nt < NT; ++nt)
+#pragma unroll
+      for (int q = 0; q < 4; ++q) ps[nt][q] = pq[nt][q] = 0.f;
+    int out_run = 0;
+    typedef float xk_f4 __attribute__((ext_vector_type(4)));
+    auto send_block = [&](int row, int d) __attribute__((always_inline)) {
+      const int tx = (row & 1) ? ((d < 2 ? txY0 : txY8) + (d & 1) * 4 * SLOTB) : ((d < 2 ? txX01 : txX23) + (d & 1) * 4 * SLOTB);
+#pragma unroll
+      for (int nt = 0; nt < NT; ++nt)
+        if (!(XK_ABL & 128))
+          *reinterpret_cast<xk_f4*>(smem + tx + nt * 1024) =
+              xk_f4{acc[d][nt][4 * row], acc[d][nt][4 * row + 1], acc[d][nt][4 * row + 2], acc[d][nt][4 * row + 3]};
+    };
+#pragma unroll
+    for (int row = 0; row < ((XK_ABL & 524288) ? 0 : 4); ++row) {
+      if (row == 0) {
+#pragma unroll
+        for (int d = 0; d < MT; ++d) send_block(0, d);
+      }
+      if (!(XK_ABL & 65536)) ff_barrier();
+      xk_f4 mv[4][NT];
+#pragma unroll
+      for (int c = 0; c < 4; ++c)
+#pragma unroll
+        for (int nt = 0; nt < NT; ++nt) {
+          if (XK_ABL & 131072) mv[c][nt] = xk_f4{acc[c % MT][nt][4 * row], acc[c % MT][nt][4 * row + 1], acc[c % MT][nt][4 * row + 2], acc[c % MT][nt][4 * row + 3]};
+          else mv[c][nt] = *reinterpret_cast<const xk_f4*>(smem + ((row & 1) ? rxY : rxX) + c * SLOTB + nt * 1024);
+        }
+#pragma unroll
+      for (int jj = 0; jj < 4; ++jj) {
+        float y1[NT];
+#pragma unroll
+        for (int nt = 0; nt < NT; ++nt) {
+          const float bs = (bv[nt] + tv[nt]) * a_out_scale;
+          const float m0 = mv[0][nt][jj], m1 = mv[1][nt][jj], m2 = mv[2][nt][jj], m3 = mv[3][nt][jj];
+          const float y0 = (m0 + m1) + m2;
+          y1[nt] = (m1 - m2) - m3;
+          float v;
+          if constexpr (RES) v = fmaf(y0, ka, fmaf(rs[row][2 * jj][nt], a_out_scale, bs));
+          else v = fmaf(y0, ka, bs);
+          if (!(XK_ABL & 8)) __builtin_amdgcn_raw_buffer_store_b32(__float_as_uint(v), out_r, out_voff + nt * 128, out_run, 0);
+          if (!(XK_ABL & 262144)) { ps[nt][(jj & 1) * 2] += v; pq[nt][(jj & 1) * 2] = fmaf(v, v, pq[nt][(jj & 1) * 2]); }
+        }
+        XW_SADD(out_run, out_col);
+#pragma unroll
+        for (int nt = 0; nt < NT; ++nt) {
+          const float bs = (bv[nt] + tv[nt]) * a_out_scale;
+          float v;
+          if constexpr (RES) v = fmaf(y1[nt], ka, fmaf(rs[row][2 * jj + 1][nt], a_out_scale, bs));
+          else v = fmaf(y1[nt], ka, bs);
+          if (!(XK_ABL & 8)) __builtin_amdgcn_raw_buffer_store_b32(__float_as_uint(v), out_r, out_voff + nt * 128, out_run, 0);
+          if (!(XK_ABL & 262144)) { ps[nt][(jj & 1) * 2 + 1] += v; pq[nt][(jj & 1) * 2 + 1] = fmaf(v, v, pq[nt][(jj & 1) * 2 + 1]); }
+        }
+        if (jj != 3) XW_SADD(out_run, out_col);
+        else if (row != 3) XW_SADD(out_run, out_row);
+        XW_FENCE();
+        if (row < 3 && jj < MT) send_block(row + 1, jj);
+        XW_FENCE();
+      }
+    }
+    if (a_stats) {
+      const int tidf = wave * 64 + lf;
+      float vs[NT], vq[NT];
+#pragma unroll
+      for (int nt = 0; nt < NT; ++nt) {
+        vs[nt] = (ps[nt][0] + ps[nt][1]) + (ps[nt][2] + ps[nt][3]);
+        vq[nt] = (pq[nt][0] + pq[nt][1]) + (pq[nt][2] + pq[nt][3]);
+        vs[nt] = e_valid ? vs[nt] : 0.f;
+        vq[nt] = e_valid ? vq[nt] : 0.f;
+        vs[nt] += __shfl_xor(vs[nt], 32);
+        vq[nt] += __shfl_xor(vq[nt], 32);
+        if (lf < 32) {
+          red[(wave * NT * 32 + nt * 32 + lf) * 2 + 0] = vs[nt];
+          red[(wave * NT * 32 + nt * 32 + lf) * 2 + 1] = vq[nt];
+        }
+      }
+      ff_barrier();
+      if (tidf < NT * 32) {
+        double sm = 0.0, sq = 0.0;
+#pragma unroll
+        for (int wv = 0; wv < 4; ++wv) {
+          sm += (double)red[(wv * NT * 32 + tidf) * 2 + 0];
+          sq += (double)red[(wv * NT * 32 + tidf) * 2 + 1];
+        }
+        double* dst = a_stats + ((size_t)e_tile * kCout + e_ng * NT * 32 + tidf) * 2;
+        dst[0] = sm;
+        dst[1] = sq;
+      }
+    }
+  };
+
+  Tile tc = tile_at(0), tn = tile_at(1);
+  Geom gc = geom_of(tc), gn = gc;
+  const int NSTB = (Cin / 16) * STB;
+
+  src_of(tc, 0);
+#pragma unroll
+  for (int j = 0; j < NSLOT; ++j) { req_a(j, gc); req_b(j, gc); }
+  req_norm(tc, 0);
+  w_begin(tc.ng * NSTB);
+  {
+    cvt_prep_half(0); cvt_prep_half(1);
+    req_norm(tc, 1);
+    src_of(tc, 1);
+    xk_static_for<NFULL>([&](auto o) __attribute__((always_inline)) { full_op(J0{}, o, gc, gc); });
+    req_a(0, gc); req_b(0, gc);
+    xk_static_for<NFULL>([&](auto o) __attribute__((always_inline)) { full_op(J1{}, o, gc, gc); });
+    req_a(1, gc); req_b(1, gc);
+    if constexpr (NSLOT == 3) {
+      xk_static_for<NFULL>([&](auto o) __attribute__((always_inline)) { full_op(J2{}, o, gc, gc); });
+      req_a(2, gc); req_b(2, gc);
+    }
+#pragma unroll
+    for (int j = 0; j < NSLOT; ++j) s_dst[j] ^= XTOG;
+    cvt_prep_half(0); cvt_prep_half(1);
+    xk_static_for<NMATH>([&](auto o) __attribute__((always_inline)) { math_op(J0{}, o, gc); });
+#pragma unroll
+    for (int i = 0; i < WPT; ++i) ld_w(w0[i], i);
+    w_next_tap();
+#pragma unroll
+    for (int i = 0; i < WPT; ++i) ld_w(w1[i], i);
+    w_next_tap();
+  }
+  ff_barrier();
+#pragma unroll
+  for (int m = 0; m < MT; ++m) { rd_x(xh[m], xb_cur, 0, m, 0); rd_x(xl[m], xb_cur, 0, m, 1); }
+
+  auto unit = [&](auto pos_tag, auto first_tag, int s) __attribute__((always_inline)) {
+    constexpr int POS = decltype(pos_tag)::value;
+    constexpr bool FIRST = decltype(first_tag)::value;
+    const Tile& tx = POS == 2 ? tn : tc;
+    const Tile& tl = POS >= 1 ? tn : tc;
+    const Geom& gx = POS == 2 ? gn : gc;
+    const Geom& gl = POS >= 1 ? gn : gc;
+    const int sl = POS == 0 ? s + 2 : POS - 1;
+    xk_static_for<3>([&](auto r_tag) __attribute__((always_inline)) {
+      constexpr int R = decltype(r_tag)::value;
+      XW_FENCE();
+      if constexpr (R == 2) { if (!(XK_ABL & 64)) ff_barrier(); }
+      XW_FENCE();
+      if constexpr (R == 0) src_of(tl, sl);
+      if constexpr (R == 1 && POS == 2) w_begin(tn.ng * NSTB);
+      constexpr int NOPS = R == 0 ? 8 + NFULL : R == 1 ? NFULL : 2 + NMATH;
+      xk_static_for<GP>([&](auto g_tag) __attribute__((always_inline)) {
+        constexpr int g = decltype(g_tag)::value;
+        XW_FENCE();
+        if constexpr (FIRST && R == 0 && g < NA) mm_first(g);
+        else if constexpr (R == 0) mm0(g / NA, g % NA);
+        else if constexpr (R == 1) mm1(g / NA, g % NA);
+        else mm2(g / NA, g % NA);
+        XW_FENCE();
+        if constexpr (S::rd_xl(g)) rd_x(xl[g / NT], R == 2 ? xb_nxt : xb_cur, (R + 1) % 3, g / NT, 1);
+        if constexpr (S::rd_xh(g)) rd_x(xh[(g - 2 * PB) / NT], R == 2 ? xb_nxt : xb_cur, (R + 1) % 3, (g - 2 * PB) / NT, 0);
+        if constexpr (S::slot_req(g) && R < NSLOT) { req_a(R, gl); req_b(R, gl); }
+        if constexpr (S::ld_w(g)) {
+          if constexpr (R == 0) ld_w(w2[g - PB], g - PB);
+          else if constexpr (R == 1) ld_w(w0[g - PB], g - PB);
+          else ld_w(w1[g - PB], g - PB);
+          if constexpr (g == PB + WPT - 1) w_next_tap();
+        }
+        if constexpr (R == 0 && g == 2 && POS == 1) epi_setup(tc);
+        if constexpr (R == (MT == 4 ? 1 : 0) && g == PB + PB / 2) req_norm(tl, sl);
+        if constexpr (R == 2 && POS == 2 && g == PB) epi_loads(tc);
+        if constexpr (MT == 4) {
+          constexpr int o0 = S::first_op(NOPS, g), o1 = S::first_op(NOPS, g + 1);
+          xk_static_for<o1 - o0>([&](auto d_tag) __attribute__((always_inline)) {
+            constexpr int o = o0 + decltype(d_tag)::value;
+            if constexpr (R == 0) {
+              if constexpr (o < 8) write_op(J0{}, std::integral_constant<int, o>{});
+              else full_op(J1{}, std::integral_constant<int, o - 8>{}, gx, gl);
+            } else if constexpr (R == 1) {
+              full_op(J2{}, std::integral_constant<int, o>{}, gx, gl);
+            } else {
+              if constexpr (o < 2) cvt_prep_half(o);
+              else math_op(J0{}, std::integral_constant<int, o - 2>{}, gl);
+            }
+          });
+        } else {
+          constexpr int NSEQ = 8 + NFULL + 2 + NMATH;
+          static_assert(S::first_op3(NSEQ, 2, 0) >= 8 + NFULL && S::first_op3(NSEQ, 1, 0) >= 8 + NPRE, "conv_xk: the half-height stage's sequence");
+          constexpr int o0 = S::first_op3(NSEQ, R, g), o1 = S::first_op3(NSEQ, R, g + 1);
+          xk_static_for<o1 - o0>([&](auto d_tag) __attribute__((always_inline)) {
+            constexpr int o = o0 + decltype(d_tag)::value;
+            if constexpr (o < 8) write_op(J0{}, std::integral_constant<int, o>{});
+            else if constexpr (o < 8 + NFULL) full_op(J1{}, std::integral_constant<int, o - 8>{}, gx, gl);
+            else if constexpr (o < 10 + NFULL) cvt_prep_half(o - 8 - NFULL);
+            else math_op(J0{}, std::integral_constant<int, o - 10 - NFULL>{}, gl);
+          });
+        }
+        constexpr int RG0 = MT == 4 ? 2 * PB : PB;
+        if constexpr (RES && POS == 2 && R == 2 && g >= RG0) {
+          constexpr int per = (8 * NT + GP - RG0 - 1) / (GP - RG0);
+#pragma unroll
+          for (int e = (g - RG0) * per; e < (g - RG0 + 1) * per && e < 8 * NT; ++e) req_res(e);
+        }
+      });
+    });
+    XW_FENCE();
+#pragma unroll
+    for (int j = 0; j < NSLOT; ++j) s_dst[j] ^= XTOG;
+    xb_cur ^= XTOG;
+    xb_nxt ^= XTOG;
+    ex_dead ^= XTOG;
+  };
+  using P0 = std::integral_constant<int, 0>;
+  using P1 = std::integral_constant<int, 1>;
+  using P2 = std::integral_constant<int, 2>;
+  using Yes = std::true_type;
+  using No = std::false_type;
+
+  for (int it = 0; it < n_my; ++it) {
+#ifdef CSD_FF_TUNE
+    if (it == 1) XW_WALL(28);
+    if (it == 2) XW_WALL(29);
+    if (it == 1 && a_dbg && tid == 0) a_dbg[blockIdx.x * 32 + 26] = clock64();
+    if (it == 2 && a_dbg && tid == 0) a_dbg[blockIdx.x * 32 + 27] = clock64();
+#endif
+    unit(P0{}, Yes{}, 0);
+    for (int s = 1; s + 2 < NS; ++s) unit(P0{}, No{}, s);
+    gn = geom_of(tn);
+    unit(P1{}, No{}, NS - 2);
+    unit(P2{}, No{}, NS - 1);
+    epilogue();
+    tc = tn;
+    gc = gn;
+    tn = tile_at(it + 2);
+  }
+  XW_WALL(31);
+}
+#undef XK_WALK_MT
+#undef XK_WALK_SPLIT
```

Result: faster. 1.644 images/sec (median of 6 runs) (+1.5%).
